# eryxcoop/acvm-backend-plonky2

Hardware: AMD Instinct MI355X
Metric: prove latency (ms) + proofs/sec at 2^20 LDE rows, 1 GPU(s): value = proofs/sec, witness resident in HBM, 4 proof(s) in flight per GPU; latency_ms_single_proof = lone resident proof; *_host_witness = p2gpu_prove from host RAM (PCIe inside the call) (higher is better)
Workload: dtype u64; 1 GPU; synth(d=17,sha): 131072 gates -> 2^20 LDE rows, 234 wires / 80 routed, KeccakGoldilocksConfig, rate 8, cap 2^4, 28 queries, 16 PoW bits (BASELINE configs[2] shape); degree_bits=17, lde_rows=1048576, mix=sha, public_inputs=0, in_flight_per_gpu=4, proof_bytes=170972

## Files before the change

### acvm-backend-plonky2_amd/__init__.py

```python
from .prover import (
    CircuitData,
    WitnessPlan,
    build_blob,
    VerifierCircuitData,
    ProofWithPublicInputs,
    P2GpuError,
    device_info,
    peer_access,
    init,
    host_array,
    host_free,
    ifft_batch,
    lde_batch,
    commit_values,
    hash_rows,
    field_selftest,
    lib_path,
    load_library,
)
from .synth import make_circuit, synth_lib_path
from . import parallel
from . import translate
from . import acir
```

### acvm-backend-plonky2_amd/csrc/circuit.hpp

```cpp
#pragma once
#include "internal.hpp"
#include "poseidon.hpp"
#include "../../include/p2gpu.h"
#include <cstring>
#include <map>
#include <string>
#include <vector>

#include <exception>

struct p2gpu_circuit;
namespace p2 {

void set_err(const char *fmt, ...);
std::string last_error_copy();
void last_error_restore(const std::string &s);

struct HostHasher {
  int kind = 0;
  const gl_t *prc = nullptr;
};
extern thread_local HostHasher g_hh;
inline size_t hh_bytes() { return g_hh.kind ? 32 : 25; }
inline void sponge_permute(gl_t st[12]) {
// ... 16 lines not shown
    } else {
      poseidon_hash_no_pad_host(v, n, d.w, g_hh.prc);
    }
    return d;
  }
  if (n * 8 <= 25) {
    for (size_t i = 0; i < n; i++) d.w[i] = v[i];
    return d;
  }
  uint64_t h[4];
  keccak256_words(v, n, h);
  return dig_from_state(h);
}
inline dig_t node_digest(const dig_t &l, const dig_t &r) {
  if (!g_hh.kind) return keccak_two_to_one(l, r);
  gl_t st[12] = {l.w[0], l.w[1], l.w[2], l.w[3], r.w[0], r.w[1], r.w[2], r.w[3], 0, 0, 0, 0};
  poseidon_permute_host(st, g_hh.prc);
  dig_t d;
  for (int i = 0; i < 4; i++) d.w[i] = st[i];
  return d;
}

struct Challenger {
  gl_t state[12];
  gl_t in[8];
  int n_in = 0;
  gl_t out[8];
  int n_out = 0;
  Challenger() { memset(state, 0, sizeof state); }
  void duplex() {
    for (int i = 0; i < n_in; i++) state[i] = in[i];
    n_in = 0;
    sponge_permute(state);
    for (int i = 0; i < 8; i++) out[i] = state[i];
    n_out = 8;
  }
  void observe(gl_t e) {
    n_out = 0;
    in[n_in++] = e;
    if (n_in == 8) duplex();
  }
  void observe_digest(const dig_t &d) {
    gl_t e[4];
    digest_elems(d, e);
    for (int i = 0; i < 4; i++) observe(e[i]);
  }
  void observe_cap(const std::vector<dig_t> &cap) {
    for (auto &d : cap) observe_digest(d);
  }
  void observe_ext(ext_t e) {
    observe(e.c0);
    observe(e.c1);
  }
  gl_t get() {
    if (n_in != 0 || n_out == 0) duplex();
    return out[--n_out];
  }
  ext_t get_ext() {
    gl_t a = get();
    gl_t b = get();
    return ext_make(a, b);
  }
};

inline dig_t host_hash_no_pad(const std::vector<gl_t> &v) {
  if (g_hh.kind) {
    dig_t d;
    poseidon_hash_no_pad_host(v.data(), v.size(), d.w, g_hh.prc);
    return d;
  }
  uint64_t h[4];
  keccak256_words(v.data(), v.size(), h);
  return dig_from_state(h);
}

template <class T>
struct DBuf {
  T *p = nullptr;
  size_t count = 0;
  hipError_t alloc(size_t n) {
    count = n;
    if (n == 0) return hipSuccess;
    return hipMalloc((void **)&p, n * sizeof(T));
  }
  void release() {
    if (p) (void)hipFree(p);
    p = nullptr;
  }
};

struct PinnedArena {
  uint8_t *base = nullptr;
  size_t cap = 0, used = 0;
  hipError_t alloc(size_t bytes) {
    cap = bytes;
    used = 0;
    return hipHostMalloc((void **)&base, bytes, hipHostMallocDefault);
  }
  void release() {
    if (base) (void)hipHostFree(base);
    base = nullptr;
  }
  void reset() { used = 0; }
  template <class T> T *take(size_t n) {
    const size_t off = (used + 63) & ~(size_t)63, bytes = n * sizeof(T);
    if (!base || off + bytes > cap) return nullptr;
    used = off + bytes;
    return (T *)(base + off);
  }
};

struct Batch {
  uint32_t cols = 0, d = 0;
  uint32_t ncl = 0;
  CosetMap cm;
  DBuf<gl_t> coeffs;
  DBuf<gl_t> lde;
  DBuf<dig_t> dig;
  std::vector<size_t> level_off;
  std::vector<dig_t> cap;
  void release() {
    coeffs.release();
    lde.release();
    dig.release();
  }
};

struct KernelStat {
  double ms = 0, bytes = 0;
  uint64_t launches = 0;
};
struct PendingEv {
  const char *name;
  double bytes;
  hipEvent_t a, b;
};


struct CircuitState {
  uint32_t d, W, R, NC, num_selectors, K, QF, rate_bits, cap_h, pow_bits, num_queries, n_steps, arity[8];
  uint32_t num_gates, num_pi, flags, PP, nchunks;
  uint32_t hasher = 0;
  size_t n, N;
  uint32_t C;
  std::vector<GateDesc> gates;
  std::vector<gl_t> k_is;
  std::vector<uint8_t> blob_prefix;
  uint32_t nterms = 0, max_gate_constraints = 0;
  uint32_t gate_groups = 1;
  uint32_t half_slots = 0;
  uint32_t gate_groups_half = 1;
  uint32_t sums_groups = 1;
  int half_gates = 1;
  bool half_auto = false;
  gl_t half_cross[16];
  DBuf<gl_t> hsum, htmp_a, htmp_b;
  int device = 0;
  hipStream_t stream = nullptr;
  hipStream_t copy_stream = nullptr;
  std::vector<hipEvent_t> copy_events;
  bool wires_ntt_done = false;
  bool wires_hash_done = false;
  DBuf<uint64_t> hash_state;
  DBuf<uint32_t> wire_nz;
  DBuf<gl_t> wire_scalar;
  uint32_t sparse_row = UINT32_MAX;
  SparseRows sparse_rows;
  DBuf<gl_t> sparse_coeffs, sparse_lde;
  DBuf<gl_t> sparse_partial;
  DBuf<uint32_t> wire_nzlist;
  DBuf<uint32_t> wire_clean;
  int zero_columns = 1;
  bool structured_off = false;
  uint32_t last_dense = 0;
  uint32_t gate_wires = 0;
  int virtual_columns = 1;
  DBuf<gl_t> tw_fwd, tw_inv, scale, inv_scale, d_kis, d_sigmas, fri_scale, qconst;
  DBuf<gl_t> l0_lde;
  DBuf<GateDesc> d_gates;
  DBuf<uint8_t> d_row_gate;
  DBuf<gl_t> d_gconsts, d_prc;
  DBuf<gl_t> d_prc_hash;
  NttPlan *plan_inv = nullptr, *plan_fwd = nullptr;
  std::vector<NttPlan *> fri_plans;
  Batch cs, wires, zp, quot;
  dig_t circuit_digest;
  gl_t poseidon_rc[360];
  gl_t poseidon_rc_gate[360];
  DBuf<gl_t> wires_vals, zp_vals, cp, scan_tmp, apow, qvals, qtmp, pw, partial, ext_apow, f01, f01v, fv;
  std::vector<DBuf<gl_t>> fri_coef, fri_vals;
  std::vector<Batch> fri_trees;
  DBuf<unsigned long long> pow_result;
  PinnedArena pin;
  uint64_t *tail_stage = nullptr;
  DBuf<uint64_t> gather_ptrs;
  DBuf<gl_t> gather_out;
  size_t gather_cap = 0;
  std::vector<uint64_t> h_ptrs;
  std::vector<uint8_t> h_out;
  int shard_rank = 0, shard_world = 1;
  p2gpu_allgather_fn shard_fn = nullptr;
  void *shard_ctx = nullptr;
  void *rccl_comm = nullptr;
  int shard_exercise = 0;
  int shard_zs = 0;
  int shard_reduce = 0;
  int shard_intt = 0;
  DBuf<gl_t> xchg_recv;
  std::vector<p2gpu_circuit *> group;
  struct PeerGroup *peer = nullptr;
  uint64_t pow_hint = UINT64_MAX;
  int profile = 0;
  int self_check = 1;
  int blocking_sync = 0;
  hipEvent_t sync_event = nullptr;
  std::map<std::string, KernelStat> kstats;
  std::vector<PendingEv> pending;
  std::vector<hipEvent_t> event_pool;
};

}

#define P2GPU_CATCH                                                   \
  catch (const std::exception &e) {                                   \
    p2::set_err("internal error: %s", e.what());                      \
    return P2GPU_E_DEVICE;                                            \
  }                                                                   \
  catch (...) {                                                       \
    p2::set_err("internal error");                                    \
    return P2GPU_E_DEVICE;                                            \
  }

struct p2gpu_circuit : p2::CircuitState {};

namespace p2 {
extern void (*g_circuit_release)(p2gpu_circuit *);
void use_hasher(const p2gpu_circuit *c);
void shard_assemble_cap(int world, unsigned rate_bits, size_t cap_per, const dig_t *gathered, std::vector<dig_t> &cap);
int circuit_parse(const uint8_t *blob, size_t len, p2gpu_circuit *c, size_t *off, const uint8_t **cap_in);
const char *gate_validate(uint32_t kind, const uint32_t p[4], uint32_t W, uint32_t gate_consts, uint64_t *wires_used,
                          uint32_t *consts_used);
uint32_t gate_num_constraints(uint32_t kind, const uint32_t p[4]);
uint32_t gate_degree(uint32_t kind, const uint32_t p[4]);
struct BuildPlan {
  size_t n = 0, prefix_len = 0;
  uint32_t R = 0, num_selectors = 0, ngc = 0, NC = 0;
  std::vector<uint32_t> gstart, gend, gsel, arity;
};
int build_plan(const p2gpu_build_params *bp, const p2gpu_gate_decl *gates, uint32_t num_gates, bool have_row_constants, BuildPlan &pl);
int build_prefix(const BuildPlan &pl, const p2gpu_build_params *bp, const p2gpu_gate_decl *gates, uint32_t hasher, uint8_t *out);
bool plonk_identity_holds(const p2gpu_circuit *c, const std::vector<ext_t> &op, const gl_t *betas, const gl_t *gammas,
                          const gl_t *alphas, ext_t zeta, const gl_t pih[4]);
}
```

### acvm-backend-plonky2_amd/csrc/gl.hpp

```cpp
#pragma once
#include <cstdint>
#include <cstddef>

#if defined(__HIPCC__)
#include <hip/hip_runtime.h>
#include <type_traits>
#define P2_HD __host__ __device__ __forceinline__
#else
#define P2_HD inline
#endif

namespace p2 {

typedef uint64_t gl_t;
constexpr uint64_t GL_P = 0xFFFFFFFF00000001ULL;
constexpr uint64_t GL_EPS = 0xFFFFFFFFULL;
constexpr uint64_t GL_GEN = 14293326489335486720ULL;
constexpr uint64_t GL_ROOT_2_32 = 7277203076849721926ULL;

#ifndef P2_GL_ASM
#define P2_GL_ASM 1
#endif
#if defined(__HIP_DEVICE_COMPILE__) && P2_GL_ASM
#define P2_GL_DEV_ASM 1
#else
#define P2_GL_DEV_ASM 0
#endif

P2_HD gl_t gl_canon_c(uint64_t x) { return x >= GL_P ? x - GL_P : x; }
P2_HD gl_t gl_add_c(gl_t a, gl_t b) {
  uint64_t s = a + b;
  if (s < a || s >= GL_P) s -= GL_P;
  return s;
}
P2_HD gl_t gl_sub_c(gl_t a, gl_t b) { return a >= b ? a - b : a - b + GL_P; }
P2_HD gl_t gl_reduce128_c(uint64_t lo, uint64_t hi) {
  uint64_t hh = hi >> 32, hl = hi & GL_EPS;
  uint64_t t0 = lo - hh;
  if (lo < hh) t0 -= GL_EPS;
  uint64_t t1 = hl * GL_EPS;
  uint64_t t2 = t0 + t1;
  if (t2 < t1) t2 += GL_EPS;
  return gl_canon_c(t2);
}

#ifndef P2_HZ_A_N
#define P2_HZ_A_N 0
#endif
#ifndef P2_HZ_B_N
#define P2_HZ_B_N 0
#endif
#if P2_HZ_A_N == 0
#define P2_HZ_A ""
#elif P2_HZ_A_N == 1
#define P2_HZ_A "s_nop 0\n\t"
#else
#define P2_HZ_A "s_nop 1\n\t"
#endif
#if P2_HZ_B_N == 0
#define P2_HZ_B ""
#elif P2_HZ_B_N == 1
#define P2_HZ_B "s_nop 0\n\t"
#else
#define P2_HZ_B "s_nop 1\n\t"
#endif
#if P2_GL_DEV_ASM
P2_HD gl_t gl_join(uint32_t lo, uint32_t hi) { return ((uint64_t)hi << 32) | lo; }
P2_HD gl_t gl_canon(uint64_t x) {
  const uint64_t g = __builtin_amdgcn_uicmpl(x, GL_P - 1, 34 );
  uint32_t r0, r1;
  uint64_t junk;
  asm("s_nop 1\n\t"
      "v_subb_co_u32 %0, %2, %3, 0, %5\n\t"
      "v_addc_co_u32 %1, %2, %4, 0, %5"
      : "=&v"(r0), "=&v"(r1), "=&s"(junk)
      : "v"((uint32_t)x), "v"((uint32_t)(x >> 32)), "s"(g));
  return gl_join(r0, r1);
}
P2_HD gl_t gl_sub(gl_t a, gl_t b) {
  uint32_t d0, d1;
  uint64_t k;
  asm("v_sub_co_u32 %0, vcc, %3, %5\n\t"
      "v_subb_co_u32 %1, vcc, %4, %6, vcc\n\t"
      "v_addc_co_u32 %0, %2, %0, 0, vcc\n\t"
      P2_HZ_A "s_andn2_b64 vcc, vcc, %2\n\t" P2_HZ_B
      "v_subb_co_u32 %1, vcc, %1, 0, vcc"
      : "=&v"(d0), "=&v"(d1), "=&s"(k)
      : "v"((uint32_t)a), "v"((uint32_t)(a >> 32)), "v"((uint32_t)b), "v"((uint32_t)(b >> 32))
      : "vcc", "scc");
  return gl_join(d0, d1);
}
P2_HD gl_t gl_add(gl_t a, gl_t b) {
  uint32_t s0, s1;
  uint64_t c;
  asm("v_add_co_u32 %0, vcc, %3, %5\n\t"
      "v_addc_co_u32 %1, %2, %4, %6, vcc"
      : "=&v"(s0), "=&v"(s1), "=&s"(c)
      : "v"((uint32_t)a), "v"((uint32_t)(a >> 32)), "v"((uint32_t)b), "v"((uint32_t)(b >> 32))
      : "vcc");
  const uint64_t m = c | __builtin_amdgcn_uicmpl(gl_join(s0, s1), GL_P - 1, 34);
  uint32_t r0, r1;
  uint64_t k;
  asm("v_subb_co_u32 %0, %2, %3, 0, %5\n\t"
      P2_HZ_A "s_andn2_b64 %2, %5, %2\n\t" P2_HZ_B
      "v_addc_co_u32 %1, %2, %4, 0, %2"
      : "=&v"(r0), "=&v"(r1), "=&s"(k)
      : "v"(s0), "v"(s1), "s"(m)
      : "scc");
  return gl_join(r0, r1);
}
P2_HD uint64_t gl_reduce_words_nc(uint32_t w0, uint32_t w1, uint32_t w2, uint32_t w3) {
  uint32_t r0, r1, y0;
  uint64_t cy, k;
  asm("v_add_co_u32 %1, vcc, %6, %7\n\t"
      "v_addc_co_u32 %2, %3, %7, %8, vcc\n\t"
      "v_addc_co_u32 %1, vcc, %1, 0, vcc\n\t"
      "v_sub_co_u32 %0, vcc, %5, %2\n\t"
      "v_subb_co_u32 %1, vcc, %1, 0, vcc\n\t"
      "v_subb_co_u32 %1, %4, %1, 0, %3\n\t"
      P2_HZ_A "s_or_b64 vcc, vcc, %4\n\t" P2_HZ_B
      "v_addc_co_u32 %0, %4, %0, 0, vcc\n\t"
      P2_HZ_A "s_andn2_b64 vcc, vcc, %4\n\t" P2_HZ_B
      "v_subb_co_u32 %1, vcc, %1, 0, vcc"
      : "=&v"(r0), "=&v"(r1), "=&v"(y0), "=&s"(cy), "=&s"(k)
      : "v"(w0), "v"(w1), "v"(w2), "v"(w3)
      : "vcc", "scc");
  return gl_join(r0, r1);
}
P2_HD gl_t gl_reduce_words(uint32_t w0, uint32_t w1, uint32_t w2, uint32_t w3) { return gl_canon(gl_reduce_words_nc(w0, w1, w2, w3)); }
P2_HD gl_t gl_reduce128(uint64_t lo, uint64_t hi) {
  return gl_reduce_words((uint32_t)lo, (uint32_t)(lo >> 32), (uint32_t)hi, (uint32_t)(hi >> 32));
}
P2_HD gl_t gl_reduce_add_eps(uint32_t w0, uint32_t w1, uint32_t w2) {
  uint32_t r0, r1, t0, t1;
  uint64_t k;
  asm("v_sub_co_u32 %2, vcc, 0, %7\n\t"
      "v_subbrev_co_u32 %3, vcc, 0, %7, vcc\n\t"
      "v_add_co_u32 %0, vcc, %5, %2\n\t"
      "v_addc_co_u32 %1, vcc, %6, %3, vcc\n\t"
      "v_subb_co_u32 %0, %4, %0, 0, vcc\n\t"
      P2_HZ_A "s_andn2_b64 vcc, vcc, %4\n\t" P2_HZ_B
      "v_addc_co_u32 %1, vcc, %1, 0, vcc"
      : "=&v"(r0), "=&v"(r1), "=&v"(t0), "=&v"(t1), "=&s"(k)
      : "v"(w0), "v"(w1), "v"(w2)
      : "vcc", "scc");
  return gl_canon(gl_join(r0, r1));
}
P2_HD gl_t gl_reduce_eps_sub(uint32_t z, uint32_t h0, uint32_t h1) {
  uint32_t r0, r1, t0, t1;
  uint64_t k;
  asm("v_sub_co_u32 %2, vcc, 0, %7\n\t"
      "v_subbrev_co_u32 %3, vcc, 0, %7, vcc\n\t"
      "v_sub_co_u32 %0, vcc, %2, %5\n\t"
      "v_subb_co_u32 %1, vcc, %3, %6, vcc\n\t"
      "v_addc_co_u32 %0, %4, %0, 0, vcc\n\t"
      P2_HZ_A "s_andn2_b64 vcc, vcc, %4\n\t" P2_HZ_B
      "v_subb_co_u32 %1, vcc, %1, 0, vcc"
      : "=&v"(r0), "=&v"(r1), "=&v"(t0), "=&v"(t1), "=&s"(k)
      : "v"(h0), "v"(h1), "v"(z)
      : "vcc", "scc");
  return gl_canon(gl_join(r0, r1));
}
#else
P2_HD gl_t gl_canon(uint64_t x) { return gl_canon_c(x); }
P2_HD gl_t gl_add(gl_t a, gl_t b) { return gl_add_c(a, b); }
P2_HD gl_t gl_sub(gl_t a, gl_t b) { return gl_sub_c(a, b); }
P2_HD gl_t gl_reduce128(uint64_t lo, uint64_t hi) { return gl_reduce128_c(lo, hi); }
#endif
#if defined(__HIPCC__)
template <class T>
__device__ __forceinline__ T ld_uniform(const T *p) {
#if defined(__HIP_DEVICE_COMPILE__)
  typedef const T __attribute__((address_space(4))) *cptr;
  return *(cptr)(uintptr_t)p;
#else
  return *p;
#endif
}
#endif
P2_HD gl_t gl_neg(gl_t a) { return a ? GL_P - a : 0; }
P2_HD gl_t gl_dbl(gl_t a) { return gl_add(a, a); }

#if defined(__HIP_DEVICE_COMPILE__)
__device__ __forceinline__ void gl_mul128(uint64_t a, uint64_t b, uint64_t &lo, uint64_t &hi) {
  const uint32_t a0 = (uint32_t)a, a1 = (uint32_t)(a >> 32), b0 = (uint32_t)b, b1 = (uint32_t)(b >> 32);
  uint64_t p0, m, p3, cdummy, carry;
  uint32_t r1, r2, r3;
  asm("v_mad_u64_u32 %0, %3, %5, %6, 0\n\t"
      "v_mad_u64_u32 %1, %3, %5, %8, 0\n\t"
      "v_mad_u64_u32 %2, %3, %7, %8, 0\n\t"
      "v_mad_u64_u32 %1, %4, %7, %6, %1"
      : "=&v"(p0), "=&v"(m), "=&v"(p3), "=&s"(cdummy), "=&s"(carry)
      : "v"(a0), "v"(b0), "v"(a1), "v"(b1));
  asm("v_add_co_u32 %0, vcc, %3, %4\n\t"
      "v_addc_co_u32 %1, vcc, %5, %6, vcc\n\t"
      "v_addc_co_u32 %2, vcc, %7, 0, vcc\n\t"
      "v_addc_co_u32 %2, vcc, %2, 0, %8"
      : "=&v"(r1), "=&v"(r2), "=&v"(r3)
      : "v"((uint32_t)(p0 >> 32)), "v"((uint32_t)m), "v"((uint32_t)p3), "v"((uint32_t)(m >> 32)),
        "v"((uint32_t)(p3 >> 32)), "s"(carry)
      : "vcc");
  lo = ((uint64_t)r1 << 32) | (uint32_t)p0;
  hi = ((uint64_t)r3 << 32) | r2;
}
#endif
P2_HD gl_t gl_mul(gl_t a, gl_t b) {
#if defined(__HIP_DEVICE_COMPILE__)
  uint64_t lo, hi;
  gl_mul128(a, b, lo, hi);
#else
  unsigned __int128 x = (unsigned __int128)a * b;
  uint64_t lo = (uint64_t)x, hi = (uint64_t)(x >> 64);
#endif
  return gl_reduce128(lo, hi);
}
P2_HD gl_t gl_sqr(gl_t a) { return gl_mul(a, a); }
#if defined(__HIP_DEVICE_COMPILE__) && P2_GL_DEV_ASM
__device__ __forceinline__ uint64_t gl_mul_nc(uint64_t a, uint64_t b) {
  uint64_t lo, hi;
  gl_mul128(a, b, lo, hi);
  return gl_reduce_words_nc((uint32_t)lo, (uint32_t)(lo >> 32), (uint32_t)hi, (uint32_t)(hi >> 32));
}
__device__ __forceinline__ uint64_t gl_reduce128_nc(uint64_t lo, uint64_t hi) {
  return gl_reduce_words_nc((uint32_t)lo, (uint32_t)(lo >> 32), (uint32_t)hi, (uint32_t)(hi >> 32));
}
#else
P2_HD uint64_t gl_mul_nc(uint64_t a, uint64_t b) { return gl_mul(gl_canon(a), gl_canon(b)); }
P2_HD uint64_t gl_reduce128_nc(uint64_t lo, uint64_t hi) { return gl_reduce128(lo, hi); }
#endif
P2_HD gl_t gl_mul_add(gl_t a, gl_t b, gl_t c) {
#if defined(__HIP_DEVICE_COMPILE__)
  uint64_t lo, hi;
  gl_mul128(a, b, lo, hi);
  lo += c;
  hi += lo < c;
#else
  unsigned __int128 x = (unsigned __int128)a * b + c;
  uint64_t lo = (uint64_t)x, hi = (uint64_t)(x >> 64);
#endif
  return gl_reduce128(lo, hi);
}
P2_HD uint64_t gl_mul_add_nc(uint64_t a, uint64_t b, gl_t c) {
#if defined(__HIP_DEVICE_COMPILE__)
  uint64_t lo, hi;
  gl_mul128(a, b, lo, hi);
  lo += c;
  hi += lo < c;
  return gl_reduce128_nc(lo, hi);
#else
  return gl_mul_add(gl_canon(a), gl_canon(b), c);
#endif
}
P2_HD gl_t gl_mul_small(gl_t a, uint32_t k) {
#if defined(__HIP_DEVICE_COMPILE__)
  uint64_t lo = a * (uint64_t)k;
  uint64_t hi = __umul64hi(a, (uint64_t)k);
#else
  unsigned __int128 x = (unsigned __int128)a * k;
  uint64_t lo = (uint64_t)x, hi = (uint64_t)(x >> 64);
#endif
  uint64_t t1 = hi * GL_EPS;
  uint64_t t2 = lo + t1;
  if (t2 < t1) t2 += GL_EPS;
  return gl_canon(t2);
}
#if defined(__HIPCC__)
struct Acc160 {
  uint32_t w[5];
  __device__ __forceinline__ void clear() { w[0] = w[1] = w[2] = w[3] = w[4] = 0; }
  __device__ __forceinline__ void mac(gl_t a, gl_t c) {
#if defined(__HIP_DEVICE_COMPILE__)
    uint64_t lo, hi;
    gl_mul128(a, c, lo, hi);
    asm("v_add_co_u32 %0, vcc, %0, %5\n\t"
        "v_addc_co_u32 %1, vcc, %1, %6, vcc\n\t"
        "v_addc_co_u32 %2, vcc, %2, %7, vcc\n\t"
        "v_addc_co_u32 %3, vcc, %3, %8, vcc\n\t"
        "v_addc_co_u32 %4, vcc, 0, %4, vcc"
        : "+v"(w[0]), "+v"(w[1]), "+v"(w[2]), "+v"(w[3]), "+v"(w[4])
        : "v"((uint32_t)lo), "v"((uint32_t)(lo >> 32)), "v"((uint32_t)hi), "v"((uint32_t)(hi >> 32))
        : "vcc");
#else
    (void)a; (void)c;
#endif
  }
  __device__ __forceinline__ gl_t value() const {
    const gl_t r = gl_reduce128(((uint64_t)w[1] << 32) | w[0], ((uint64_t)w[3] << 32) | w[2]);
    return gl_sub(r, (uint64_t)w[4] << 32);
  }
};
#endif
P2_HD gl_t gl_pow(gl_t b, uint64_t e) {
  gl_t r = 1;
  while (e) {
    if (e & 1) r = gl_mul(r, b);
    b = gl_sqr(b);
    e >>= 1;
  }
  return r;
}
P2_HD gl_t gl_sqr_n(gl_t a, int k) {
  for (int i = 0; i < k; i++) a = gl_mul(a, a);
  return a;
}
P2_HD gl_t gl_inv(gl_t a) {
  const gl_t e2 = gl_mul(gl_mul(a, a), a);
  const gl_t e4 = gl_mul(gl_sqr_n(e2, 2), e2);
  const gl_t e8 = gl_mul(gl_sqr_n(e4, 4), e4);
  const gl_t e16 = gl_mul(gl_sqr_n(e8, 8), e8);
  const gl_t e24 = gl_mul(gl_sqr_n(e16, 8), e8);
  const gl_t e28 = gl_mul(gl_sqr_n(e24, 4), e4);
  const gl_t e30 = gl_mul(gl_sqr_n(e28, 2), e2);
  const gl_t e31 = gl_mul(gl_mul(e30, e30), a);
  const gl_t e32 = gl_mul(gl_mul(e31, e31), a);
  return gl_mul(gl_sqr_n(e31, 33), e32);
}
P2_HD gl_t gl_root(unsigned k) {
  gl_t g = GL_ROOT_2_32;
  for (unsigned i = k; i < 32; i++) g = gl_sqr(g);
  return g;
}
// ... 107 lines not shown
```

### acvm-backend-plonky2_amd/csrc/handle.hip

```cpp
#include "prover_internal.hpp"
#include <functional>

using namespace p2;

namespace {

void release_for_destroy(p2gpu_circuit *c) {
  for (p2gpu_circuit *m : c->group) {
    m->peer = nullptr;
    release_for_destroy(m);
    delete m;
  }
  c->group.clear();
  if (c->peer && c->shard_rank == 0) {
    for (auto e : c->peer->recv_free) if (e) (void)hipEventDestroy(e);
    for (auto e : c->peer->sent) if (e) (void)hipEventDestroy(e);
    delete c->peer;
  }
  c->peer = nullptr;
  (void)hipSetDevice(c->device);
  if (c->stream) (void)hipStreamSynchronize(c->stream);
  if (c->rccl_comm) (void)rccl().CommDestroy((ncclComm_t)c->rccl_comm);
  c->rccl_comm = nullptr;
  circuit_release(c);
}
struct ReleaseHook {
  ReleaseHook() { p2::g_circuit_release = release_for_destroy; }
} g_release_hook;

struct Scratch {
  std::vector<void *> ptrs;
  hipStream_t st = nullptr;
  ~Scratch() {
    for (void *p : ptrs) (void)hipFree(p);
    if (st) (void)hipStreamDestroy(st);
  }
  template <class T> T *alloc(size_t n) {
    void *p = nullptr;
    if (hipMalloc(&p, (n ? n : 1) * sizeof(T)) != hipSuccess) return nullptr;
    ptrs.push_back(p);
    return (T *)p;
  }
};

}

namespace p2 {

int g_device = -1;
std::vector<int> g_peer_access;
std::vector<int> g_devices;

void circuit_release(p2gpu_circuit *c) {
  c->tw_fwd.release(); c->tw_inv.release(); c->scale.release(); c->inv_scale.release(); c->d_kis.release();
  c->d_sigmas.release(); c->fri_scale.release(); c->d_gates.release(); c->qconst.release(); c->l0_lde.release();
  c->d_row_gate.release(); c->d_gconsts.release(); c->d_prc.release(); c->d_prc_hash.release();
  c->hsum.release(); c->htmp_a.release(); c->htmp_b.release();
  c->cs.release(); c->wires.release(); c->zp.release(); c->quot.release();
  c->wires_vals.release(); c->zp_vals.release(); c->cp.release(); c->scan_tmp.release();
  c->apow.release(); c->qvals.release(); c->qtmp.release(); c->pw.release(); c->partial.release();
  c->ext_apow.release(); c->f01.release(); c->f01v.release(); c->fv.release();
  for (auto &b : c->fri_coef) b.release();
  for (auto &b : c->fri_vals) b.release();
  for (auto &b : c->fri_trees) b.release();
  c->hash_state.release();
  c->wire_nz.release();
  c->wire_nzlist.release();
  c->wire_clean.release();
  c->wire_scalar.release(); c->sparse_coeffs.release(); c->sparse_lde.release(); c->sparse_partial.release();
  c->pin.release();
  if (c->sync_event) (void)hipEventDestroy(c->sync_event);
  c->sync_event = nullptr;
  if (c->tail_stage) (void)hipHostFree(c->tail_stage);
  c->tail_stage = nullptr;
  c->pow_result.release(); c->gather_ptrs.release(); c->gather_out.release(); c->xchg_recv.release();
  ntt_plan_destroy(c->plan_inv);
  ntt_plan_destroy(c->plan_fwd);
  for (auto *p : c->fri_plans)
    if (p != c->plan_fwd) ntt_plan_destroy(p);
  c->plan_inv = c->plan_fwd = nullptr;
  c->fri_plans.clear();
  for (auto e : c->event_pool) (void)hipEventDestroy(e);
  for (auto e : c->copy_events) (void)hipEventDestroy(e);
  if (c->copy_stream) (void)hipStreamDestroy(c->copy_stream);
  if (c->stream) (void)hipStreamDestroy(c->stream);
}

int ensure_device() {
  if (g_device >= 0) return 0;
  int cnt = 0;
  hipError_t e = hipGetDeviceCount(&cnt);
  if (e != hipSuccess || cnt == 0) {
    set_err("no HIP device available (%s); libp2gpu has no CPU fallback", e == hipSuccess ? "count=0" : hipGetErrorString(e));
    return P2GPU_E_DEVICE;
  }
  int dev = 0;
  (void)hipGetDevice(&dev);
  g_device = dev;
  g_devices.assign(1, dev);
  g_peer_access.assign(1, -1);
  return 0;
}

}


namespace {

#define CK(e, what)                                       \
  do {                                                    \
    const hipError_t e_ = (e);                            \
    if (e_ != hipSuccess) {                               \
      set_err("%s: %s", what, hipGetErrorString(e_));     \
      return P2GPU_E_DEVICE;                              \
    }                                                     \
  } while (0)

void schedule_gates(p2gpu_circuit *c) {
  c->nterms = c->K + c->K * c->nchunks + c->max_gate_constraints;
  auto cost = [](const GateDesc &g) { return g.kind == G_POSEIDON ? 0u : 4u * g.num_constraints + 8u; };
  const uint32_t perm_cost = (uint32_t)env_uint("P2GPU_PERM_COST", 8u * c->R + 100u);
  uint32_t total = 0;
  for (auto &g : c->gates) total += cost(g);
  c->gate_groups = env_uint("P2GPU_GATE_GROUPS", total > 2 * perm_cost ? 4u : 1u) == 4 ? 4u : 1u;
  uint32_t load[4] = {perm_cost, 0, 0, 0};
  std::vector<uint32_t> order(c->gates.size());
  for (size_t i = 0; i < order.size(); i++) order[i] = (uint32_t)i;
  std::sort(order.begin(), order.end(), [&](uint32_t x, uint32_t y) { return cost(c->gates[x]) > cost(c->gates[y]); });
  for (uint32_t gi : order) {
    uint32_t best = 0;
    for (uint32_t q = 1; q < 4; q++)
      if (load[q] < load[best]) best = q;
    c->gates[gi].pad = c->gate_groups == 4 ? best : 0;
    load[best] += cost(c->gates[gi]);
  }
  uint64_t half_constraints = 0;
  if (env_flag("P2GPU_HALF_GATES", true) && c->d >= 6 && c->rate_bits == 3)
    for (auto &g : c->gates)
      if (g.kind != G_POSEIDON && g.num_constraints >= 48 && gate_degree(g.kind, g.p) <= 4 && c->half_slots < 64) {
        g.pad |= (++c->half_slots) << 16;
        half_constraints += g.num_constraints;
      }
  c->half_auto = (half_constraints << c->d) >= ((uint64_t)12 << 20);
  if (c->half_slots) {
    auto cost_main = [&](const GateDesc &g) { return gate_half_slot(g) ? 8u : cost(g); };
    uint32_t rest = 0;
    for (auto &g : c->gates) rest += cost_main(g);
    c->gate_groups_half = env_uint("P2GPU_GATE_GROUPS_HALF", rest > 2 * perm_cost ? 4u : 1u) == 4 ? 4u : 1u;
    uint32_t lm[4] = {perm_cost, 0, 0, 0}, ls[4] = {0, 0, 0, 0};
    c->sums_groups = env_uint("P2GPU_SUMS_GROUPS", c->half_slots >= 2 ? 4u : 1u) == 4 ? 4u : 1u;
    for (uint32_t gi : order) {
      GateDesc &g = c->gates[gi];
      uint32_t bm = 0, bs = 0;
      for (uint32_t q = 1; q < 4; q++) {
        if (lm[q] < lm[bm]) bm = q;
        if (ls[q] < ls[bs]) bs = q;
      }
      if (c->gate_groups_half == 4) g.pad |= bm << 4;
      lm[bm] += cost_main(g);
      if (gate_half_slot(g)) {
        if (c->sums_groups == 4) g.pad |= bs << 8;
        ls[bs] += cost(g);
      }
    }
  }
}

int make_streams(p2gpu_circuit *c) {
  if (poseidon_upload_constants()) { set_err("uploading Poseidon constants failed"); return P2GPU_E_DEVICE; }
  CK(hipStreamCreateWithFlags(&c->stream, hipStreamNonBlocking), "hipStreamCreate");
  CK(hipStreamCreateWithFlags(&c->copy_stream, hipStreamNonBlocking), "hipStreamCreate");
  return P2GPU_OK;
}

int make_root_tables(p2gpu_circuit *c) {
  hipStream_t st = c->stream;
  const size_t n = c->n;
  const uint32_t d = c->d, K = c->K, C = c->C;
  const size_t half = n >= 2 ? n / 2 : 1;
  CK(c->tw_fwd.alloc(half), "alloc tw");
  CK(c->tw_inv.alloc(half), "alloc tw");
  CK(c->scale.alloc((size_t)C * n), "alloc scale");
  CK(c->inv_scale.alloc((size_t)C * n), "alloc scale");
  CK(c->fri_scale.alloc((size_t)C * n), "alloc scale");
  CK(c->d_kis.alloc(c->R), "alloc kis");
  CK(c->d_sigmas.alloc((size_t)c->R * n), "alloc sigmas");
  CK(c->d_gates.alloc(c->num_gates ? c->num_gates : 1), "alloc gates");
  gl_t wn = gl_root(d), wN = gl_root(d + c->rate_bits);
  c->plan_inv = ntt_plan_create(st, d, NttDir::ToCoeffs);
  c->plan_fwd = ntt_plan_create(st, d, NttDir::ToValues);
  if (!c->plan_inv || !c->plan_fwd) { set_err("ntt plan allocation failed"); return P2GPU_E_DEVICE; }
  fill_powers(st, c->tw_fwd.p, wn, (uint32_t)half);
  fill_powers(st, c->tw_inv.p, gl_inv(wn), (uint32_t)half);
  fill_coset_scale(st, c->scale.p, GL_GEN, wN, d, C, 1);
  fill_coset_scale(st, c->inv_scale.p, gl_inv(GL_GEN), gl_inv(wN), d, C, 1);
  if (c->half_slots) {
    const size_t per = (size_t)4 * c->half_slots * K * n;
    CK(c->hsum.alloc(2 * per), "alloc gate sums");
    CK(c->htmp_a.alloc(per), "alloc gate sums");
    CK(c->htmp_b.alloc(per), "alloc gate sums");
    const gl_t w8 = gl_root(3), quarter = gl_inv(4);
    for (int mo = 0; mo < 4; mo++)
      for (int m = 0; m < 4; m++) {
        const gl_t base = gl_pow(w8, (uint64_t)((2 * mo + 1 - 2 * m + 16) % 8));
        gl_t acc = 0, pw = 1;
        for (int j = 0; j < 4; j++) {
          acc = gl_add(acc, pw);
          pw = gl_mul(pw, base);
        }
        c->half_cross[4 * mo + m] = gl_mul(acc, quarter);
      }
  }
  CK(c->qconst.alloc(24), "alloc qconst");
  {
    gl_t qc[24];
    memset(qc, 0, sizeof qc);
    gl_t wC = gl_root(c->rate_bits), gn = gl_pow(GL_GEN, n);
    for (uint32_t r = 0; r < C; r++) {
      qc[r] = gl_mul(GL_GEN, gl_pow(wN, r));
      qc[8 + r] = gl_sub(gl_mul(gn, gl_pow(wC, r)), 1);
      qc[16 + r] = gl_inv(qc[8 + r]);
    }
    CK(hipMemcpy(c->qconst.p, qc, sizeof qc, hipMemcpyHostToDevice), "copy qconst");
    CK(c->l0_lde.alloc((size_t)C * n), "alloc L0 table");
    fill_l0_table(st, c->qconst.p, c->tw_fwd.p, 0, d, C, gl_inv((gl_t)n), c->l0_lde.p);
  }
  return P2GPU_OK;
}

int tables_from_blob(p2gpu_circuit *c, const gl_t *constants, const gl_t *sigmas) {
  const size_t n = c->n;
  const uint32_t ngc = c->NC - c->num_selectors;
  CK(hipMemcpyAsync(c->d_sigmas.p, sigmas, 8 * (size_t)c->R * n, hipMemcpyHostToDevice, c->stream), "copy sigmas");
  std::vector<uint8_t> rg(n, 0);
  for (size_t row = 0; row < n; row++) {
    uint32_t gi = 0;
    for (uint32_t s = 0; s < c->num_selectors; s++) {
      gl_t v = constants[(size_t)s * n + row];
      if (c->num_selectors == 1 || v != 0xFFFFFFFFULL) gi = (uint32_t)v;
    }
    if (gi >= c->num_gates) { set_err("selector column holds an unknown gate index"); return P2GPU_E_BLOB; }
    rg[row] = (uint8_t)gi;
    if (c->sparse_row == UINT32_MAX && c->gates[gi].kind == G_PUBLIC_INPUT) c->sparse_row = (uint32_t)row;
  }
  c->sparse_rows = SparseRows();
  if (c->sparse_row != UINT32_MAX) {
    c->sparse_rows.row[c->sparse_rows.count++] = c->sparse_row;
    for (size_t row = 0; row < n && c->sparse_rows.count < MAX_SPARSE_ROWS; row++)
      if (c->gates[rg[row]].kind == G_POSEIDON) c->sparse_rows.row[c->sparse_rows.count++] = (uint32_t)row;
  }
  CK(hipMemcpy(c->d_row_gate.p, rg.data(), n, hipMemcpyHostToDevice), "copy row_gate");
  if (ngc)
    CK(hipMemcpy(c->d_gconsts.p, constants + (size_t)c->num_selectors * n, 8 * (size_t)ngc * n, hipMemcpyHostToDevice), "copy gconsts");
  return P2GPU_OK;
}

int alloc_proof_buffers(p2gpu_circuit *c) {
  hipStream_t st = c->stream;
  const size_t n = c->n;
  const uint32_t d = c->d, K = c->K, C = c->C;
  const uint32_t ncs = c->NC + c->R, nzp = K * (1 + c->PP), nq = K * c->QF;
  const uint32_t nall = ncs + c->W + nzp + nq;
  if (batch_alloc(c, c->cs, ncs) || batch_alloc(c, c->wires, c->W) || batch_alloc(c, c->zp, nzp) || batch_alloc(c, c->quot, nq)) return P2GPU_E_DEVICE;
  CK(c->wires_vals.alloc((size_t)c->W * n), "alloc wires");
  CK(c->wire_nz.alloc(c->W), "alloc wire flags");
  CK(c->wire_nzlist.alloc(c->W + 1), "alloc wire flags");
  CK(c->wire_clean.alloc(c->W), "alloc wire flags");
  CK(hipMemsetAsync(c->wire_clean.p, 0, sizeof(uint32_t) * c->W, c->stream), "clear wire flags");
  CK(c->wire_scalar.alloc((size_t)MAX_SPARSE_ROWS * c->W), "alloc wire flags");
  if (c->sparse_row != UINT32_MAX) {
    const uint32_t nr = c->sparse_rows.count;
    CK(c->sparse_coeffs.alloc((size_t)nr * n), "alloc sparse basis");
// ... 267 lines not shown


int p2gpu_circuit_create_on(const uint8_t *blob, size_t len, int device_id, p2gpu_circuit **out_c) try {
  if (!blob || !out_c) return P2GPU_E_ARG;
  if (int rc = ensure_device()) return rc;
  if (std::find(g_devices.begin(), g_devices.end(), device_id) == g_devices.end()) {
    set_err("p2gpu_circuit_create_on: device %d is not in the list given to p2gpu_init", device_id);
    return P2GPU_E_ARG;
  }
  const int rc = circuit_create_one(blob, len, device_id, out_c);
  (void)hipSetDevice(g_device);
  return rc;
} P2GPU_CATCH

static int circuit_make(const std::function<int(int, p2gpu_circuit **)> &one, p2gpu_circuit **out_c) {
  if (g_devices.size() <= 1) return one(g_device, out_c);
  const int n = (int)g_devices.size();
  std::vector<p2gpu_circuit *> hs(n, nullptr);
  std::vector<int> rcs(n, 0);
  std::vector<std::string> errs(n);
  {
    std::vector<std::thread> th;
    for (int q = 0; q < n; q++)
      th.emplace_back([&, q] {
        rcs[q] = one(g_devices[q], &hs[q]);
        if (rcs[q]) errs[q] = p2gpu_last_error();
      });
    for (auto &t : th) t.join();
  }
  (void)hipSetDevice(g_device);
  auto drop = [&](int rc, const std::string &msg) {
    for (auto *h : hs)
      if (h) {
        h->peer = nullptr;
        p2gpu_circuit_destroy(h);
      }
    set_err("%s", msg.c_str());
    return rc;
  };
  for (int q = 0; q < n; q++)
    if (rcs[q]) return drop(rcs[q], errs[q]);
  for (int q = 0; q < n; q++) {
    if (int rc = shard_args_ok(hs[q], q, n)) return drop(rc, p2gpu_last_error());
    if (int rc = shard_layout(hs[q], q, n)) return drop(rc, p2gpu_last_error());
  }
  PeerGroup *pg = new PeerGroup();
  pg->n = n;
  pg->cs = hs;
  pg->recv_free.assign(n, nullptr);
  pg->sent.assign(n, nullptr);
  pg->proof_scratch.resize(n);
  pg->send_ptr.resize(n);
  pg->recv_ptr.resize(n);
  for (int q = 0; q < n; q++) {
    (void)hipSetDevice(hs[q]->device);
    if (hipEventCreateWithFlags(&pg->recv_free[q], hipEventDisableTiming) != hipSuccess ||
        hipEventCreateWithFlags(&pg->sent[q], hipEventDisableTiming) != hipSuccess) {
      for (int k = 0; k <= q; k++) {
        (void)hipSetDevice(hs[k]->device);
        if (pg->recv_free[k]) (void)hipEventDestroy(pg->recv_free[k]);
        if (pg->sent[k]) (void)hipEventDestroy(pg->sent[k]);
        hs[k]->peer = nullptr;
      }
      (void)hipSetDevice(g_device);
      delete pg;
      return drop(P2GPU_E_DEVICE, "hipEventCreate failed");
    }
    hs[q]->peer = pg;
  }
  (void)hipSetDevice(g_device);
  for (int q = 1; q < n; q++) hs[0]->group.push_back(hs[q]);
  *out_c = hs[0];
  return P2GPU_OK;
}

int p2gpu_circuit_create(const uint8_t *blob, size_t len, p2gpu_circuit **out_c) try {
  if (!blob || !out_c) return P2GPU_E_ARG;
  if (int rc = ensure_device()) return rc;
  return circuit_make([&](int device, p2gpu_circuit **h) { return circuit_create_one(blob, len, device, h); }, out_c);
} P2GPU_CATCH


int p2gpu_circuit_build_on(const p2gpu_build_params *bp, const p2gpu_gate_decl *gates, uint32_t num_gates, const uint32_t *row_gate,
                           const uint64_t *row_constants, const uint32_t *copies, size_t num_copies, uint32_t hasher, int device_id,
                           p2gpu_circuit **out_c) try {
  BuildCall b;
  if (int rc = build_call_prepare(b, bp, gates, num_gates, row_gate, row_constants, copies, num_copies, hasher, out_c)) return rc;
  if (int rc = ensure_device()) return rc;
  if (std::find(g_devices.begin(), g_devices.end(), device_id) == g_devices.end()) {
    set_err("p2gpu_circuit_build_on: device %d is not in the list given to p2gpu_init", device_id);
    return P2GPU_E_ARG;
  }
  const int rc = circuit_build_one(b, device_id, out_c);
  (void)hipSetDevice(g_device);
  return rc;
} P2GPU_CATCH

int p2gpu_circuit_build(const p2gpu_build_params *bp, const p2gpu_gate_decl *gates, uint32_t num_gates, const uint32_t *row_gate,
                        const uint64_t *row_constants, const uint32_t *copies, size_t num_copies, uint32_t hasher, p2gpu_circuit **out_c) try {
  BuildCall b;
  if (int rc = build_call_prepare(b, bp, gates, num_gates, row_gate, row_constants, copies, num_copies, hasher, out_c)) return rc;
  if (int rc = ensure_device()) return rc;
  return circuit_make([&](int device, p2gpu_circuit **h) { return circuit_build_one(b, device, h); }, out_c);
} P2GPU_CATCH

int p2gpu_circuit_export_blob(const p2gpu_circuit *cc, uint8_t *out, size_t *len) try {
  if (!cc || !len) return P2GPU_E_ARG;
  if (int rc = prover_handle(cc)) return rc;
  p2gpu_circuit *c = const_cast<p2gpu_circuit *>(cc);
  const size_t n = c->n, nsel = c->num_selectors, ngc = c->NC - c->num_selectors;
  const size_t need = c->blob_prefix.size() + 8 * ((size_t)c->NC + c->R) * n;
  if (!out || *len < need) {
    const bool probe = out == nullptr;
    *len = need;
    if (probe) return P2GPU_OK;
    set_err("blob buffer too small: need %zu bytes", need);
    return P2GPU_E_BUFFER;
  }
  HIP_TRY(hipSetDevice(c->device));
  Scratch S;
  gl_t *sel = S.alloc<gl_t>(nsel * n);
  if (!sel) { set_err("hipMalloc failed"); (void)hipSetDevice(g_device); return P2GPU_E_DEVICE; }
  build_selector_columns(c->stream, c, sel);
  memcpy(out, c->blob_prefix.data(), c->blob_prefix.size());
  uint8_t *q = out + c->blob_prefix.size();
  hipError_t e = hipMemcpyAsync(q, sel, 8 * nsel * n, hipMemcpyDeviceToHost, c->stream);
  if (e == hipSuccess && ngc) e = hipMemcpyAsync(q + 8 * nsel * n, c->d_gconsts.p, 8 * ngc * n, hipMemcpyDeviceToHost, c->stream);
  if (e == hipSuccess) e = hipMemcpyAsync(q + 8 * (size_t)c->NC * n, c->d_sigmas.p, 8 * (size_t)c->R * n, hipMemcpyDeviceToHost, c->stream);
  const hipError_t e2 = hipStreamSynchronize(c->stream);
  (void)hipSetDevice(g_device);
  HIP_TRY(e);
  HIP_TRY(e2);
  *len = need;
  return P2GPU_OK;
} P2GPU_CATCH




int p2gpu_circuit_set(p2gpu_circuit *c, const char *key, uint64_t value) try {
  if (!c || !key) return P2GPU_E_ARG;
  if (int rc = prover_handle(c)) return rc;
  for (p2gpu_circuit *m : c->group)
    if (int rc = p2gpu_circuit_set(m, key, value)) return rc;
  HIP_TRY(hipSetDevice(c->device));
  std::string k(key);
  if (k == "pow_hint") c->pow_hint = value;
  else if (k == "self_check") c->self_check = (int)value;
  else if (k == "shard_exercise") c->shard_exercise = (int)value;
  else if (k == "shard_intt") c->shard_intt = (int)value;
  else if (k == "shard_reduce") c->shard_reduce = (int)value;
  else if (k == "shard_zs") c->shard_zs = (int)value;
  else if (k == "half_gates") c->half_gates = (int)value;
  else if (k == "blocking_sync") c->blocking_sync = (int)value;
  else if (k == "virtual_columns") {
    c->virtual_columns = (int)value;
    if (c->wire_clean.p) HIP_TRY(hipMemsetAsync(c->wire_clean.p, 0, sizeof(uint32_t) * c->W, c->stream));
  }
  else if (k == "zero_columns") {
    c->zero_columns = (int)value;
    c->structured_off = false;
    if (c->wire_clean.p) HIP_TRY(hipMemsetAsync(c->wire_clean.p, 0, sizeof(uint32_t) * c->W, c->stream));
  }
  else if (k == "profile") {
    flush_kstats(c);
    c->profile = (int)value;
    c->kstats.clear();
  } else {
    set_err("unknown knob %s", key);
    return P2GPU_E_ARG;
  }
  return P2GPU_OK;
} P2GPU_CATCH

static int shard_layout(p2gpu_circuit *c, int rank, int world) {
  HIP_TRY(hipSetDevice(c->device));
  if (c->stream) HIP_TRY(hipStreamSynchronize(c->stream));
  if (c->rccl_comm) {
    (void)rccl().CommDestroy((ncclComm_t)c->rccl_comm);
    c->rccl_comm = nullptr;
  }
  c->shard_rank = rank;
  c->shard_world = world;
  c->shard_fn = nullptr;
  c->shard_ctx = nullptr;
  const uint32_t ncl = c->C / (uint32_t)world;
  const size_t cap_per = ((size_t)1 << c->cap_h) >> c->rate_bits;
  CosetMap cm;
  cm.first = (uint32_t)rank;
  cm.stride = (uint32_t)world;
  Batch *bs[3] = {&c->wires, &c->zp, &c->quot};
  for (Batch *b : bs) {
    b->ncl = ncl;
    b->cm = cm;
    tree_layout(*b, ncl, c->n, cap_per);
  }
  if (c->n_steps > 0) {
    Batch &t0 = c->fri_trees[0];
    t0.ncl = ncl;
    t0.cm = cm;
    tree_layout(t0, ncl, c->n >> c->arity[0], cap_per);
  }
  if (c->wire_clean.p) HIP_TRY(hipMemsetAsync(c->wire_clean.p, 0, sizeof(uint32_t) * c->W, c->stream));
  c->xchg_recv.release();
  HIP_TRY(c->xchg_recv.alloc(std::max({(size_t)world * c->gather_cap, (size_t)c->K * c->C * c->n, (size_t)2 * world * c->n}) + 64));
  return P2GPU_OK;
}
static int shard_args_ok(p2gpu_circuit *c, int rank, int world) {
  if (!c || world < 1 || rank < 0 || rank >= world || (c->C % (uint32_t)world) != 0) {
    set_err("bad shard configuration: rank %d of %d (cosets %u)", rank, world, c ? c->C : 0u);
    return P2GPU_E_ARG;
  }
  if (int rc = prover_handle(c)) return rc;
  return P2GPU_OK;
}

static int not_a_group(const p2gpu_circuit *c) {
  if (c && c->peer) { set_err("this handle is a device group of one process (p2gpu_init with several ids): its sharding is fixed"); return P2GPU_E_ARG; }
  return P2GPU_OK;
}
int p2gpu_circuit_set_shard(p2gpu_circuit *c, int rank, int world, p2gpu_allgather_fn fn, void *ctx) try {
  if (int rc = not_a_group(c)) return rc;
  if (int rc = shard_args_ok(c, rank, world)) return rc;
  if (world > 1 && !fn) { set_err("a host all-gather callback is needed for world > 1 (or use p2gpu_circuit_set_shard_rccl)"); return P2GPU_E_ARG; }
  if (int rc = shard_layout(c, rank, world)) return rc;
  c->shard_fn = fn;
  c->shard_ctx = ctx;
  return P2GPU_OK;
} P2GPU_CATCH

int p2gpu_shard_unique_id(uint8_t id_out[128]) try {
  if (!id_out) return P2GPU_E_ARG;
  if (int rc = ensure_device()) return rc;
  if (!rccl().ok) { set_err("librccl.so.1 could not be loaded"); return P2GPU_E_DEVICE; }
  ncclUniqueId id;
  static_assert(sizeof id == 128, "ncclUniqueId is 128 bytes");
  RCCL_TRY(rccl().GetUniqueId(&id));
  memcpy(id_out, &id, sizeof id);
  return P2GPU_OK;
} P2GPU_CATCH

int p2gpu_circuit_set_shard_rccl(p2gpu_circuit *c, int rank, int world, const uint8_t id_in[128]) try {
  if (int rc = not_a_group(c)) return rc;
  if (int rc = shard_args_ok(c, rank, world)) return rc;
  if (!id_in) return P2GPU_E_ARG;
  if (!rccl().ok) { set_err("librccl.so.1 could not be loaded"); return P2GPU_E_DEVICE; }
  if (int rc = shard_layout(c, rank, world)) return rc;
  ncclUniqueId id;
  memcpy(&id, id_in, sizeof id);
  ncclComm_t comm = nullptr;
  RCCL_TRY(rccl().CommInitRank(&comm, world, id, rank));
  c->rccl_comm = (void *)comm;
  return P2GPU_OK;
} P2GPU_CATCH

int p2gpu_kernel_stats(p2gpu_circuit *c, char *names, double *ms, double *bytes, uint64_t *launches, int cap) try {
  if (!c) return P2GPU_E_ARG;
  if (int rc = prover_handle(c)) return rc;
  (void)hipSetDevice(c->device);
  (void)hipStreamSynchronize(c->stream);
  flush_kstats(c);
  int i = 0;
  for (auto &kv : c->kstats) {
    if (i >= cap) break;
    snprintf(names + 64 * i, 64, "%s", kv.first.c_str());
    ms[i] = kv.second.ms;
    bytes[i] = kv.second.bytes;
    launches[i] = kv.second.launches;
    i++;
  }
  return i;
} P2GPU_CATCH

int p2gpu_ifft_batch(const uint64_t *vals, size_t ncols, unsigned d, uint64_t *coeffs_out) try {
  if (int rc = ensure_device()) return rc;
  if (!vals || !coeffs_out || d > 24) return P2GPU_E_ARG;
  Scratch S;
  HIP_TRY(hipStreamCreate(&S.st));
  size_t n = (size_t)1 << d, half = n >= 2 ? n / 2 : 1;
  gl_t *a = S.alloc<gl_t>(ncols * n), *b = S.alloc<gl_t>(ncols * n), *tw = S.alloc<gl_t>(half);
  if (!a || !b || !tw) { set_err("hipMalloc failed"); return P2GPU_E_DEVICE; }
  HIP_TRY(hipMemcpyAsync(a, vals, 8 * ncols * n, hipMemcpyHostToDevice, S.st));
  NttPlan *plan = ntt_plan_create(S.st, d, NttDir::ToCoeffs);
  if (!plan) { set_err("hipMalloc failed"); return P2GPU_E_DEVICE; }
  ntt_batch(S.st, plan, a, b, (uint32_t)ncols, 1, nullptr, gl_inv((gl_t)n), false);
  bitrev_cols(S.st, b, a, d, (uint32_t)ncols);
  hipError_t e1 = hipMemcpyAsync(coeffs_out, a, 8 * ncols * n, hipMemcpyDeviceToHost, S.st);
  hipError_t e2 = hipStreamSynchronize(S.st);
  ntt_plan_destroy(plan);
  HIP_TRY(e1);
  HIP_TRY(e2);
  return P2GPU_OK;
} P2GPU_CATCH

int p2gpu_lde_batch(const uint64_t *coeffs, size_t ncols, unsigned d, unsigned rate_bits, uint64_t *lde_out) try {
  if (int rc = ensure_device()) return rc;
  if (!coeffs || !lde_out || d > 24 || rate_bits > 3) return P2GPU_E_ARG;
  Scratch S;
  HIP_TRY(hipStreamCreate(&S.st));
  size_t n = (size_t)1 << d, half = n >= 2 ? n / 2 : 1;
  uint32_t C = 1u << rate_bits;
  gl_t *a = S.alloc<gl_t>(ncols * n), *b = S.alloc<gl_t>(ncols * n), *tw = S.alloc<gl_t>(half);
  gl_t *scale = S.alloc<gl_t>(C * n), *lde = S.alloc<gl_t>(C * ncols * n);
  if (!a || !b || !tw || !scale || !lde) { set_err("hipMalloc failed"); return P2GPU_E_DEVICE; }
  HIP_TRY(hipMemcpyAsync(a, coeffs, 8 * ncols * n, hipMemcpyHostToDevice, S.st));
  bitrev_cols(S.st, a, b, d, (uint32_t)ncols);
  NttPlan *plan = ntt_plan_create(S.st, d, NttDir::ToValues);
  if (!plan) { set_err("hipMalloc failed"); return P2GPU_E_DEVICE; }
  fill_coset_scale(S.st, scale, GL_GEN, gl_root(d + rate_bits), d, C, 1);
  ntt_batch(S.st, plan, b, lde, (uint32_t)ncols, C, scale, 1, false);
  std::vector<gl_t> tmp(C * ncols * n);
  hipError_t e1 = hipMemcpyAsync(tmp.data(), lde, 8 * tmp.size(), hipMemcpyDeviceToHost, S.st);
  hipError_t e2 = hipStreamSynchronize(S.st);
  ntt_plan_destroy(plan);
  HIP_TRY(e1);
  HIP_TRY(e2);
  for (uint32_t r = 0; r < C; r++)
    for (size_t col = 0; col < ncols; col++)
      for (size_t k = 0; k < n; k++) lde_out[col * C * n + C * k + r] = tmp[((size_t)r * ncols + col) * n + k];
  return P2GPU_OK;
} P2GPU_CATCH

static int field_selftest_words(const uint64_t *a, const uint64_t *b, size_t n, uint64_t *bad_out, size_t words);
int p2gpu_field_selftest(const uint64_t *a, const uint64_t *b, size_t n, uint64_t bad_out[8]) { return field_selftest_words(a, b, n, bad_out, 8); }
int p2gpu_field_selftest16(const uint64_t *a, const uint64_t *b, size_t n, uint64_t bad_out[16]) { return field_selftest_words(a, b, n, bad_out, 16); }
static int field_selftest_words(const uint64_t *a, const uint64_t *b, size_t n, uint64_t *bad_out, size_t words) try {
  if (int rc = ensure_device()) return rc;
  if (!a || !b || !bad_out || n == 0 || n > ((size_t)1 << 28)) return P2GPU_E_ARG;
  Scratch S;
  HIP_TRY(hipStreamCreate(&S.st));
  uint64_t *da = S.alloc<uint64_t>(n), *db = S.alloc<uint64_t>(n);
  unsigned long long *bad = S.alloc<unsigned long long>(16);
  if (!da || !db || !bad) { set_err("hipMalloc failed"); return P2GPU_E_DEVICE; }
  HIP_TRY(hipMemcpyAsync(da, a, 8 * n, hipMemcpyHostToDevice, S.st));
  HIP_TRY(hipMemcpyAsync(db, b, 8 * n, hipMemcpyHostToDevice, S.st));
  HIP_TRY(hipMemsetAsync(bad, 0, 128, S.st));
  field_selftest(S.st, da, db, (uint32_t)n, bad);
  HIP_TRY(hipMemcpyAsync(bad_out, bad, 8 * words, hipMemcpyDeviceToHost, S.st));
  HIP_TRY(hipStreamSynchronize(S.st));
  return P2GPU_OK;
} P2GPU_CATCH

int p2gpu_hash_rows(const uint64_t *rows, size_t n_rows, size_t row_len, uint8_t *digests_out) try {
  if (int rc = ensure_device()) return rc;
  if (!rows || !digests_out) return P2GPU_E_ARG;
  Scratch S;
  HIP_TRY(hipStreamCreate(&S.st));
  gl_t *a = S.alloc<gl_t>(n_rows * row_len);
  dig_t *dg = S.alloc<dig_t>(n_rows);
  if (!a || !dg) { set_err("hipMalloc failed"); return P2GPU_E_DEVICE; }
  HIP_TRY(hipMemcpyAsync(a, rows, 8 * n_rows * row_len, hipMemcpyHostToDevice, S.st));
  hash_rows(S.st, a, n_rows, (uint32_t)row_len, dg);
  std::vector<dig_t> h(n_rows);
  HIP_TRY(hipMemcpyAsync(h.data(), dg, sizeof(dig_t) * n_rows, hipMemcpyDeviceToHost, S.st));
  HIP_TRY(hipStreamSynchronize(S.st));
  for (size_t i = 0; i < n_rows; i++) memcpy(digests_out + 25 * i, h[i].w, 25);
  return P2GPU_OK;
} P2GPU_CATCH

int p2gpu_commit_values(const uint64_t *vals, size_t ncols, unsigned d, unsigned rate_bits, unsigned cap_h,
                        uint8_t *cap_out) try {
  if (int rc = ensure_device()) return rc;
  if (!vals || !cap_out || d > 24 || rate_bits > 3 || cap_h < rate_bits || cap_h > rate_bits + d) return P2GPU_E_ARG;
  HalfBuilt own(new p2gpu_circuit());
  p2gpu_circuit *c = own.get();
  c->d = d; c->rate_bits = rate_bits; c->cap_h = cap_h; c->n = (size_t)1 << d; c->N = c->n << rate_bits;
  c->C = 1u << rate_bits; c->device = g_device; c->n_steps = 0;
  int rc = P2GPU_OK;
  size_t n = c->n, half = n >= 2 ? n / 2 : 1;
  do {
    if (hipStreamCreate(&c->stream) != hipSuccess || c->tw_fwd.alloc(half) != hipSuccess ||
        c->tw_inv.alloc(half) != hipSuccess || c->scale.alloc((size_t)c->C * n) != hipSuccess ||
        c->wires_vals.alloc(ncols * n) != hipSuccess || c->pin.alloc(((size_t)1 << 16) + 2 * (sizeof(dig_t) << cap_h)) != hipSuccess) {
      set_err("hipMalloc failed");
      rc = P2GPU_E_DEVICE;
      break;
    }
    if ((rc = batch_alloc(c, c->wires, (uint32_t)ncols))) break;
    c->plan_inv = ntt_plan_create(c->stream, d, NttDir::ToCoeffs);
    c->plan_fwd = ntt_plan_create(c->stream, d, NttDir::ToValues);
    if (!c->plan_inv || !c->plan_fwd) {
      set_err("hipMalloc failed");
      rc = P2GPU_E_DEVICE;
      break;
    }
    fill_coset_scale(c->stream, c->scale.p, GL_GEN, gl_root(d + rate_bits), d, c->C, 1);
    if (hipMemcpyAsync(c->wires_vals.p, vals, 8 * ncols * n, hipMemcpyHostToDevice, c->stream) != hipSuccess) {
      set_err("copy failed");
      rc = P2GPU_E_DEVICE;
      break;
    }
    if ((rc = batch_commit_from_values(c, c->wires, c->wires_vals.p))) break;
    for (size_t i = 0; i < c->wires.cap.size(); i++) memcpy(cap_out + 25 * i, c->wires.cap[i].w, 25);
  } while (0);
  return rc;
} P2GPU_CATCH

}
```

### acvm-backend-plonky2_amd/csrc/internal.hpp

```cpp
#pragma once
#include <hip/hip_runtime.h>
#include <cstdlib>
#include <vector>
#include "gl.hpp"
#include "keccak.hpp"
#include "gates.hpp"

namespace p2 {

constexpr int MAX_GATES = 64;
constexpr uint32_t MAX_GATE_CONSTRAINTS = 4096;
constexpr uint32_t MAX_ARITY_BITS = 4;
constexpr int MAX_CHALLENGES = 2;
constexpr int MAX_ROUTED = 128;

inline bool env_flag(const char *name, bool dflt) {
  const char *e = getenv(name);
  return e && *e ? *e != '0' : dflt;
}
inline uint64_t env_uint(const char *name, uint64_t dflt) {
  const char *e = getenv(name);
  return e ? strtoull(e, nullptr, 10) : dflt;
}

struct Prof {
  virtual void begin(const char *kernel, double algorithmic_bytes) = 0;
  virtual void end() = 0;
  virtual ~Prof() {}
};
extern thread_local Prof *g_prof;
struct ProfScope {
  ProfScope(const char *k, double bytes) { if (g_prof) g_prof->begin(k, bytes); }
  ~ProfScope() { if (g_prof) g_prof->end(); }
};

constexpr uint32_t MAX_SPARSE_ROWS = 4;
struct SparseRows {
  uint32_t row[MAX_SPARSE_ROWS] = {UINT32_MAX, UINT32_MAX, UINT32_MAX, UINT32_MAX};
  uint32_t count = 0;
};
struct ColHints {
  const uint32_t *cls = nullptr;
  const uint32_t *clean = nullptr;
  const gl_t *val = nullptr;
  const gl_t *basis = nullptr;
  bool basis_per_coset = false;
  uint32_t nrows = 1, val_stride = 0;
  size_t basis_stride = 0;
  uint32_t virt_first = UINT32_MAX;
  uint32_t dense_hint = 0;
  bool fill_only = false;
};
void column_clean_update(hipStream_t st, const uint32_t *cls, uint32_t cols, uint32_t *clean, bool after);
void column_flags(hipStream_t st, const gl_t *vals, uint32_t cols, uint32_t d, const SparseRows &rows, uint32_t *flags,
                  gl_t *scalar, uint32_t sstride);

constexpr int NTT_MAX_ROUNDS = 6;
enum class NttDir { ToCoeffs, ToValues };
struct NttPass {
  uint32_t s, a, tb, nrounds;
  uint32_t r[NTT_MAX_ROUNDS], tw_off[NTT_MAX_ROUNDS];
  bool direct = false;
  uint32_t rm = 0, rl = 0, fold_r = 0, fold_s0 = 0;
  uint32_t ftw_off = 0;
};
struct NttPlan {
  uint32_t d = 0;
  NttDir dir = NttDir::ToCoeffs;
  std::vector<NttPass> passes;
  gl_t *ptw = nullptr;
  size_t table_len = 0;
};
struct CosetMap {
  uint32_t first = 0, stride = 1;
};
NttPlan *ntt_plan_create(hipStream_t st, uint32_t d, NttDir dir);
void ntt_plan_destroy(NttPlan *p);
void ntt_batch(hipStream_t st, const NttPlan *plan, const gl_t *src, gl_t *dst, uint32_t cols, uint32_t cosets,
               const gl_t *scale, gl_t post, bool src_per_coset, CosetMap cm = CosetMap(), uint32_t stride_cols = 0,
               const ColHints *hints = nullptr);

void fill_powers(hipStream_t st, gl_t *out, gl_t root, uint32_t count);
void fill_coset_scale(hipStream_t st, gl_t *out, gl_t shift, gl_t wN, uint32_t d, uint32_t cosets, gl_t mult);

void bitrev_cols(hipStream_t st, const gl_t *in, gl_t *out, uint32_t d, uint32_t cols);
void field_selftest(hipStream_t st, const uint64_t *a, const uint64_t *b, uint32_t n, unsigned long long *bad);

struct VirtCols {
  const uint32_t *cls = nullptr;
  const gl_t *val = nullptr;
  const gl_t *basis = nullptr;
  uint32_t first = UINT32_MAX;
  uint32_t coset_first = 0, coset_stride = 1;
};
uint32_t hash_lde_leaves(hipStream_t st, const gl_t *lde, uint32_t cols, uint32_t d, uint32_t cosets, dig_t *dig, const gl_t *prc = nullptr,
                         const VirtCols *virt = nullptr, dig_t *lvl1 = nullptr, dig_t *lvl2 = nullptr);
void hash_lde_absorb(hipStream_t st, const gl_t *lde, uint32_t cols, uint32_t d, uint32_t cosets, uint32_t blk0,
                     uint32_t nblk, bool first, bool last, uint64_t *state, dig_t *dig, const VirtCols *virt = nullptr);
void hash_rows(hipStream_t st, const gl_t *rows, size_t n_rows, uint32_t row_len, dig_t *dig);
void hash_fri_leaves(hipStream_t st, const gl_t *vals, uint32_t lg_npc, uint32_t cosets, uint32_t arity_bits,
                     dig_t *dig, const gl_t *prc = nullptr);
bool tree_levels(hipStream_t st, dig_t *lvl, uint32_t cosets, uint32_t m, uint32_t cap_per, const gl_t *prc = nullptr,
                 dig_t *host_mirror = nullptr);

struct ZsArgs {
  const gl_t *wires;
  const gl_t *sigmas;
  const gl_t *k_is;
  const gl_t *sub_tw;
  uint32_t tw_shift;
  uint32_t d, R, QF, nchunks, K;
  gl_t betas[MAX_CHALLENGES], gammas[MAX_CHALLENGES];
  gl_t *cp;
  uint32_t sb;
  uint32_t row0, rows;
  gl_t *zp;
};
void zs_partial_products(hipStream_t st, const ZsArgs &a, gl_t *scan_tmp);
void zs_chunks(hipStream_t st, const ZsArgs &a);
void zs_scan_finish(hipStream_t st, const ZsArgs &a, gl_t *scan_tmp);

struct QuotArgs {
  const gl_t *cs_lde;
  const gl_t *wires_lde;
  const gl_t *zp_lde;
  const gl_t *k_is;
  const gl_t *tw;
  const gl_t *apow;
  const GateDesc *gates;
  const GateDesc *host_gates;
  gl_t *out;
  uint32_t tw_shift, d, rate_bits, W, R, NC, num_selectors, K, QF, nchunks, PP, num_gates, nterms, has_poseidon;
  uint32_t gate_groups;
  uint32_t gate_groups_half;
  uint32_t use_half;
  uint32_t nsk;
  gl_t *hsum;
  uint32_t coset_first, coset_stride, ncosets;
  gl_t betas[MAX_CHALLENGES], gammas[MAX_CHALLENGES];
  gl_t pi_hash[4];
  const gl_t *qconst;
  gl_t n_inv;
  const gl_t *l0;
};
void quotient_eval(hipStream_t st, const QuotArgs &a);
void gate_sums_eval(hipStream_t st, const QuotArgs &a, uint32_t groups);
void gate_sums_cross(hipStream_t st, const gl_t *in, const gl_t *inv_scale, gl_t *out, uint32_t d, uint32_t cols, const gl_t F[16]);
void fill_l0_table(hipStream_t st, const gl_t *qconst, const gl_t *tw, uint32_t tw_shift, uint32_t d, uint32_t cosets, gl_t n_inv, gl_t *out);
int poseidon_upload_constants();
void quotient_chunks(hipStream_t st, const gl_t *in, const gl_t *inv_scale, gl_t *out, uint32_t d, uint32_t K,
                     uint32_t rate_bits, gl_t w_inv, gl_t gn_inv, gl_t rate_inv, uint32_t world = 1);

void fill_witness(hipStream_t st, gl_t *wires, const uint8_t *row_gate, const GateDesc *gates, const gl_t *gconsts,
                  const gl_t *prc, uint32_t d, uint32_t ngc, uint32_t num_wires);

void ext_powers_bitrev2(hipStream_t st, ext_t base0, ext_t base1, uint32_t d, gl_t *out0, gl_t *out1);
void eval_columns(hipStream_t st, const gl_t *coeffs, uint32_t cols, uint32_t d, const gl_t *pw, uint32_t parts,
                  gl_t *partial , const ColHints *hints = nullptr, const gl_t *basis_partial = nullptr);
struct EvalSegs {
  struct Seg {
    const gl_t *coeffs;
    const gl_t *pw;
    gl_t *partial;
    uint32_t cols;
  } seg[6];
  uint32_t count = 0, hinted = UINT32_MAX;
  const uint32_t *cls = nullptr;
  const gl_t *val = nullptr, *basis_partial = nullptr;
};
void eval_columns_multi(hipStream_t st, const EvalSegs &S, uint32_t d, uint32_t parts, uint32_t col0 = 0, uint32_t ncols = UINT32_MAX);
void reduce_columns(hipStream_t st, const gl_t *coeffs, uint32_t cols, uint32_t d, const gl_t *apow ,
                    uint32_t j0, gl_t *acc, bool accumulate, const uint32_t *nzlist = nullptr, const gl_t *basis = nullptr,
                    const gl_t *fold = nullptr);
void compact_nonzero(hipStream_t st, const uint32_t *flags, uint32_t cols, uint32_t *list);
void sum_parts(hipStream_t st, const gl_t *parts, uint32_t nparts, size_t len, gl_t *out);
void class1_fold(hipStream_t st, const ColHints &h, uint32_t cols, const gl_t *apow, uint32_t j0, gl_t *fold);
void fri_quotient_values(hipStream_t st, const gl_t *F0, const gl_t *F1, uint32_t d, const gl_t *tw, uint32_t tw_shift,
                         ext_t zeta, ext_t gzeta, ext_t f0z, ext_t f1z, ext_t aK, gl_t *out );
void fri_fold(hipStream_t st, const gl_t *in , uint32_t d, uint32_t arity_bits, ext_t beta, gl_t *out);
void pow_search(hipStream_t st, const gl_t state[12], uint32_t pos, uint32_t pow_bits, uint64_t base, uint64_t count,
                unsigned long long *result, const gl_t *prc = nullptr);
void gather_u64(hipStream_t st, const uint64_t *addr, uint32_t count, gl_t *out);

}
```

### acvm-backend-plonky2_amd/csrc/plonk.hip

```cpp
#include "internal.hpp"
#include "gates.hpp"

namespace p2 {

__constant__ gl_t c_poseidon_rc[360];
int poseidon_upload_constants() {
  gl_t rc[360];
  poseidon_round_constants_host(rc);
  gl_t dev[360];
  poseidon_device_constants(rc, dev);
  return hipMemcpyToSymbol(HIP_SYMBOL(c_poseidon_rc), dev, sizeof dev) == hipSuccess ? 0 : -1;
}

__device__ __forceinline__ gl_t root_pow(const gl_t *tw, uint32_t shift, uint32_t d, uint32_t i) {
  uint32_t half = 1u << (d - 1);
  if (d == 0) return 1;
  return i < half ? tw[(size_t)i << shift] : gl_neg(tw[(size_t)(i - half) << shift]);
}

__device__ __forceinline__ size_t zs_idx(const ZsArgs &a, uint32_t col, uint32_t i) {
  const uint32_t cols = a.K * (a.nchunks + 1);
  return ((((size_t)(i >> a.sb) * cols + col) << a.sb) | (i & ((1u << a.sb) - 1u)));
}
__global__ __launch_bounds__(256) void zs_chunk_kernel(ZsArgs a) {
  const uint32_t n = 1u << a.d;
  const uint32_t i = a.row0 + blockIdx.x * blockDim.x + threadIdx.x;
  const uint32_t c = blockIdx.y;
  if (i >= a.row0 + a.rows) return;
  const gl_t x = root_pow(a.sub_tw, a.tw_shift, a.d, i);
  const gl_t beta = a.betas[c], gamma = a.gammas[c];
  const gl_t bx = gl_mul(beta, x);
  gl_t np[16], dp[16];
  for (uint32_t m = 0; m < a.nchunks; m++) {
    uint64_t pn = 1, pd = 1;
    for (uint32_t j = m * a.QF; j < (m + 1) * a.QF && j < a.R; j++) {
      gl_t wv = a.wires[(size_t)j * n + i];
      const gl_t wg = gl_add(wv, gamma);
      const uint64_t num = gl_mul_add_nc(bx, a.k_is[j], wg);
      const uint64_t den = gl_mul_add_nc(beta, a.sigmas[(size_t)j * n + i], wg);
      pn = gl_mul_nc(pn, num);
      pd = gl_mul_nc(pd, den);
    }
    np[m] = gl_canon(pn);
    dp[m] = gl_canon(pd);
  }
  gl_t pre[16];
  gl_t acc = 1;
  for (uint32_t m = 0; m < a.nchunks; m++) {
    pre[m] = acc;
    acc = gl_mul(acc, dp[m]);
  }
  gl_t inv = gl_inv(acc);
  gl_t rowp = 1;
  for (uint32_t m = a.nchunks; m-- > 0;) {
    gl_t di = gl_mul(inv, pre[m]);
    inv = gl_mul(inv, dp[m]);
    gl_t q = gl_mul(np[m], di);
    a.cp[zs_idx(a, c * a.nchunks + m, i)] = q;
    rowp = gl_mul(rowp, q);
  }
  a.cp[zs_idx(a, a.K * a.nchunks + c, i)] = rowp;
}

__device__ __forceinline__ gl_t block_scan_mul(gl_t v, gl_t *lds, gl_t *total) {
  const uint32_t t = threadIdx.x, nt = blockDim.x;
  lds[t] = v;
  __syncthreads();
  for (uint32_t off = 1; off < nt; off <<= 1) {
    gl_t x = lds[t];
    gl_t y = t >= off ? lds[t - off] : 1;
    __syncthreads();
    lds[t] = gl_mul(x, y);
    __syncthreads();
  }
  gl_t incl = lds[t];
  gl_t excl = t ? lds[t - 1] : 1;
  *total = lds[nt - 1];
  (void)incl;
  return excl;
}

__global__ __launch_bounds__(256) void scan_local_kernel(const ZsArgs a, uint32_t n, gl_t *local, gl_t *bsum, uint32_t nblocks) {
  __shared__ gl_t lds[256];
  const uint32_t i = blockIdx.x * blockDim.x + threadIdx.x;
  const uint32_t c = blockIdx.y;
  gl_t v = i < n ? a.cp[zs_idx(a, a.K * a.nchunks + c, i)] : 1;
  gl_t total;
  gl_t excl = block_scan_mul(v, lds, &total);
  if (i < n) local[(size_t)c * n + i] = excl;
  if (threadIdx.x == 0) bsum[(size_t)c * nblocks + blockIdx.x] = total;
}
__global__ __launch_bounds__(1024) void scan_blocks_kernel(gl_t *bsum, uint32_t nblocks) {
  __shared__ gl_t lds[1024];
  const uint32_t c = blockIdx.x;
  gl_t *b = bsum + (size_t)c * nblocks;
  const uint32_t per = (nblocks + blockDim.x - 1) / blockDim.x;
  const uint32_t lo = threadIdx.x * per;
  gl_t prod = 1;
  for (uint32_t j = lo; j < lo + per && j < nblocks; j++) prod = gl_mul(prod, b[j]);
  gl_t total;
  gl_t excl = block_scan_mul(prod, lds, &total);
  gl_t acc = excl;
  for (uint32_t j = lo; j < lo + per && j < nblocks; j++) {
    gl_t v = b[j];
    b[j] = acc;
    acc = gl_mul(acc, v);
  }
}
__global__ __launch_bounds__(256) void zs_finish_kernel(ZsArgs a, const gl_t *local, const gl_t *bpre,
                                                        uint32_t nblocks) {
  const uint32_t n = 1u << a.d;
  const uint32_t i = blockIdx.x * blockDim.x + threadIdx.x;
  const uint32_t c = blockIdx.y;
  if (i >= n) return;
  const uint32_t PP = a.nchunks - 1;
  gl_t z = gl_mul(bpre[(size_t)c * nblocks + blockIdx.x], local[(size_t)c * n + i]);
  a.zp[(size_t)c * n + i] = z;
  gl_t acc = z;
  for (uint32_t m = 0; m < PP; m++) {
    acc = gl_mul(acc, a.cp[zs_idx(a, c * a.nchunks + m, i)]);
    a.zp[((size_t)a.K + (size_t)c * PP + m) * n + i] = acc;
  }
}

void zs_chunks(hipStream_t st, const ZsArgs &a) {
  if (!a.rows) return;
  ProfScope ps("zs_chunk_kernel", 8.0 * a.K * (double)a.rows * (2.0 * a.R + a.nchunks + 1));
  hipLaunchKernelGGL(zs_chunk_kernel, dim3((a.rows + 255) / 256, a.K), dim3(256), 0, st, a);
}
void zs_scan_finish(hipStream_t st, const ZsArgs &a, gl_t *scan_tmp) {
  const uint32_t n = 1u << a.d;
  const uint32_t threads = 256;
  const uint32_t nblocks = (n + threads - 1) / threads;
  gl_t *local = scan_tmp;
  gl_t *bsum = scan_tmp + (size_t)a.K * n;
  ProfScope ps2("zs_scan_finish", 8.0 * a.K * (double)n * (2.0 * a.nchunks + 4));
  hipLaunchKernelGGL(scan_local_kernel, dim3(nblocks, a.K), dim3(threads), 0, st, a, n, local, bsum, nblocks);
  hipLaunchKernelGGL(scan_blocks_kernel, dim3(a.K), dim3(1024), 0, st, bsum, nblocks);
  hipLaunchKernelGGL(zs_finish_kernel, dim3(nblocks, a.K), dim3(threads), 0, st, a, local, bsum, nblocks);
}
void zs_partial_products(hipStream_t st, const ZsArgs &a, gl_t *scan_tmp) {
  zs_chunks(st, a);
  zs_scan_finish(st, a, scan_tmp);
}

struct Consumer {
  Acc160 acc0, acc1;
  const gl_t *ap0, *ap1;
  uint32_t t;
  __device__ __forceinline__ void emit(gl_t c) {
    acc0.mac(ap0[t], c);
    acc1.mac(ap1[t], c);
    t++;
  }
};

#ifndef P2_QUOT_WAVES
#define P2_QUOT_WAVES 6
#endif
template <bool POSEIDON, int G>
__global__ __launch_bounds__(256, P2_QUOT_WAVES) void quotient_kernel(const QuotArgs a) {
  __shared__ gl_t red[2][G > 1 ? G : 1][G > 1 ? 64 : 1];
  const uint32_t grp = G > 1 ? threadIdx.y : 0;
  const uint32_t n = 1u << a.d;
  const uint32_t k = blockIdx.x * blockDim.x + threadIdx.x;
  const uint32_t z = blockIdx.y;
  const uint32_t r = a.coset_first + z * a.coset_stride;
  if (k >= n) return;
  const uint32_t ncs = a.NC + a.R, nzp = a.K * (1 + a.PP);
  const gl_t *cs = a.cs_lde + (size_t)r * ncs * n + k;
  const gl_t *wl = a.wires_lde + (size_t)z * a.W * n + k;
  const gl_t *zl = a.zp_lde + (size_t)z * nzp * n;
  const uint32_t kn = (k + 1) & (n - 1);
  const gl_t x = gl_mul(a.qconst[r], root_pow(a.tw, a.tw_shift, a.d, k));
  Consumer out;
  out.acc0.clear();
  out.acc1.clear();
  out.ap0 = a.apow;
  out.ap1 = a.apow + a.nterms;
  out.t = 0;
  if (grp == 0) {
  const gl_t l0 = a.l0[(size_t)r * n + k];
  for (uint32_t c = 0; c < a.K; c++) out.emit(gl_mul(l0, gl_sub(zl[(size_t)c * n + k], 1)));
  {
    const gl_t bx0 = gl_mul(a.betas[0], x), bx1 = gl_mul(a.betas[1], x);
    const uint32_t t_base = out.t;
    for (uint32_t m = 0; m < a.nchunks; m++) {
      uint64_t n0, d0, n1 = 1, d1 = 1;
      {
        const uint32_t j = m * a.QF;
        const gl_t wv = wl[(size_t)j * n];
        const gl_t sg = cs[(size_t)(a.NC + j) * n];
        const gl_t kj = a.k_is[j];
        const gl_t wg0 = gl_add(wv, a.gammas[0]);
        n0 = gl_mul_add_nc(bx0, kj, wg0);
        d0 = gl_mul_add_nc(a.betas[0], sg, wg0);
        if (a.K > 1) {
          const gl_t wg1 = gl_add(wv, a.gammas[1]);
          n1 = gl_mul_add_nc(bx1, kj, wg1);
          d1 = gl_mul_add_nc(a.betas[1], sg, wg1);
        }
      }
#pragma unroll 7
      for (uint32_t j = m * a.QF + 1; j < (m + 1) * a.QF && j < a.R; j++) {
        const gl_t wv = wl[(size_t)j * n];
        const gl_t sg = cs[(size_t)(a.NC + j) * n];
        const gl_t kj = a.k_is[j];
        const gl_t wg0 = gl_add(wv, a.gammas[0]);
        n0 = gl_mul_nc(n0, gl_mul_add_nc(bx0, kj, wg0));
        d0 = gl_mul_nc(d0, gl_mul_add_nc(a.betas[0], sg, wg0));
        if (a.K > 1) {
          const gl_t wg1 = gl_add(wv, a.gammas[1]);
          n1 = gl_mul_nc(n1, gl_mul_add_nc(bx1, kj, wg1));
          d1 = gl_mul_nc(d1, gl_mul_add_nc(a.betas[1], sg, wg1));
        }
      }
      for (uint32_t c = 0; c < a.K; c++) {
        const gl_t prev = m == 0 ? zl[(size_t)c * n + k] : zl[((size_t)a.K + c * a.PP + m - 1) * n + k];
        const gl_t next = m == a.nchunks - 1 ? zl[(size_t)c * n + kn] : zl[((size_t)a.K + c * a.PP + m) * n + k];
        const gl_t term = c == 0 ? gl_sub(gl_mul(prev, n0), gl_mul(next, d0)) : gl_sub(gl_mul(prev, n1), gl_mul(next, d1));
        out.t = t_base + c * a.nchunks + m;
        out.emit(term);
      }
    }
    out.t = t_base + a.K * a.nchunks;
  }
  }
  const uint32_t t_gates = a.K + a.K * a.nchunks;
  gl_t tot0 = out.acc0.value(), tot1 = out.acc1.value();
  auto W = [&](uint32_t c) { return wl[(size_t)c * n]; };
  auto LC = [&](uint32_t i) { return cs[(size_t)(a.num_selectors + i) * n]; };
  for (uint32_t gi = 0; gi < a.num_gates; gi++) {
    const GateDesc g = a.gates[gi];
    if (g.num_constraints == 0) continue;
    if (!POSEIDON && g.kind == G_POSEIDON) continue;
    if (G > 1 && gate_group(g, a.use_half) != grp) continue;
    const gl_t s = cs[(size_t)g.sel_index * n];
    const gl_t f = gate_filter<BaseOps>(g, gi, a.num_selectors, s);
    if (const uint32_t slot1 = a.use_half ? gate_half_slot(g) : 0u) {
      const gl_t *h = a.hsum + ((size_t)((r & 1u) * 4u + (r >> 1)) * a.nsk + (size_t)(slot1 - 1) * a.K) * n + k;
      tot0 = gl_mul_add(f, h[0], tot0);
      if (a.K > 1) tot1 = gl_mul_add(f, h[n], tot1);
      continue;
    }
    out.acc0.clear();
    out.acc1.clear();
    out.t = t_gates;
    eval_gate<BaseOps, POSEIDON>(g, W, LC, a.pi_hash, c_poseidon_rc, out);
    tot0 = gl_add(tot0, gl_mul(f, out.acc0.value()));
    tot1 = gl_add(tot1, gl_mul(f, out.acc1.value()));
  }
  if constexpr (G > 1) {
    red[0][grp][threadIdx.x] = tot0;
    red[1][grp][threadIdx.x] = tot1;
    __syncthreads();
    if (grp != 0) return;
    for (int q = 1; q < G; q++) {
      tot0 = gl_add(tot0, red[0][q][threadIdx.x]);
      tot1 = gl_add(tot1, red[1][q][threadIdx.x]);
    }
  }
  const gl_t zi = a.qconst[16 + r];
  a.out[((size_t)0 * a.ncosets + z) * n + k] = gl_mul(tot0, zi);
  if (a.K > 1) a.out[((size_t)1 * a.ncosets + z) * n + k] = gl_mul(tot1, zi);
}

#ifndef P2_SUMS_WAVES
#define P2_SUMS_WAVES 8
#endif
template <int G, bool STAGE>
__global__ __launch_bounds__(256, P2_SUMS_WAVES) void gate_sums_kernel(const QuotArgs a) {
  extern __shared__ gl_t sums_stage[];
  const uint32_t grp = G > 1 ? threadIdx.y : 0;
  const uint32_t n = 1u << a.d;
  const uint32_t k = blockIdx.x * blockDim.x + threadIdx.x;
  const uint32_t m = blockIdx.y, r = 2u * m;
  if (k >= n) return;
  const uint32_t ncs = a.NC + a.R;
  const gl_t *csb = a.cs_lde + (size_t)r * ncs * n;
  const gl_t *wlb = a.wires_lde + (size_t)r * a.W * n;
  Consumer out;
  out.ap0 = a.apow;
  out.ap1 = a.apow + a.nterms;
  const uint32_t kb = k * 8u;
  auto W = [&](uint32_t c) { return *(const gl_t *)((const char *)(wlb + (size_t)c * n) + kb); };
  auto LC = [&](uint32_t i) { return *(const gl_t *)((const char *)(csb + (size_t)(a.num_selectors + i) * n) + kb); };
  for (uint32_t gi = 0; gi < a.num_gates; gi++) {
    const GateDesc g = a.gates[gi];
    const uint32_t slot1 = gate_half_slot(g);
    if (!slot1) continue;
    if (G > 1 && gate_sums_group(g) != grp) continue;
    out.acc0.clear();
    out.acc1.clear();
    out.t = a.K + a.K * a.nchunks;
    eval_gate<BaseOps, false>(g, W, LC, a.pi_hash, c_poseidon_rc, out);
    if constexpr (STAGE) {
      const uint32_t rb = blockDim.x, sk = (slot1 - 1) * a.K;
      sums_stage[sk * rb + threadIdx.x] = out.acc0.value();
      if (a.K > 1) sums_stage[(sk + 1) * rb + threadIdx.x] = out.acc1.value();
    } else {
      gl_t *h = a.hsum + ((size_t)m * a.nsk + (size_t)(slot1 - 1) * a.K) * n + k;
      h[0] = out.acc0.value();
      if (a.K > 1) h[n] = out.acc1.value();
    }
  }
  if constexpr (STAGE) {
    for (uint32_t gi = 0; gi < a.num_gates; gi++) {
      const GateDesc g = a.gates[gi];
      const uint32_t slot1 = gate_half_slot(g);
      if (!slot1 || (G > 1 && gate_sums_group(g) != grp)) continue;
      const uint32_t rb = blockDim.x, sk = (slot1 - 1) * a.K;
      gl_t *h = a.hsum + ((size_t)m * a.nsk + sk) * n + k;
      h[0] = sums_stage[sk * rb + threadIdx.x];
      if (a.K > 1) h[n] = sums_stage[(sk + 1) * rb + threadIdx.x];
    }
  }
}
struct CrossMat {
  gl_t f[4][4];
};
__global__ __launch_bounds__(256) void gate_sums_cross_kernel(const gl_t *__restrict__ in, const gl_t *__restrict__ inv_scale, gl_t *__restrict__ out,
                                                             uint32_t d, uint32_t cols, CrossMat F) {
  const uint32_t n = 1u << d;
  const uint32_t p = blockIdx.x * blockDim.x + threadIdx.x, col = blockIdx.y;
  if (p >= n) return;
  gl_t P[4];
#pragma unroll
  for (uint32_t m = 0; m < 4; m++) P[m] = gl_mul(in[((size_t)m * cols + col) * n + p], inv_scale[(size_t)(2 * m) * n + p]);
#pragma unroll
  for (uint32_t mo = 0; mo < 4; mo++) {
    Acc160 acc;
    acc.clear();
#pragma unroll
    for (uint32_t m = 0; m < 4; m++) acc.mac(F.f[mo][m], P[m]);
    out[((size_t)mo * cols + col) * n + p] = acc.value();
  }
}
void gate_sums_eval(hipStream_t st, const QuotArgs &a, uint32_t groups) {
  const uint32_t n = 1u << a.d;
  const size_t lds = (size_t)a.nsk * (groups == 4 ? 64 : 256) * sizeof(gl_t);
  static const bool stage_ok = env_flag("P2GPU_SUMS_STAGE", true);
  const bool stage = stage_ok && lds <= 24 * 1024;
  const char *name = groups == 4 ? (stage ? "gate_sums_kernel<4, true>" : "gate_sums_kernel<4, false>") : (stage ? "gate_sums_kernel<1, true>" : "gate_sums_kernel<1, false>");
  ProfScope ps(name, 8.0 * (double)n * 4 * (a.W + a.num_selectors + 1.0 * a.nsk));
  if (groups == 4) {
    if (stage) hipLaunchKernelGGL((gate_sums_kernel<4, true>), dim3(n / 64, 4), dim3(64, 4), lds, st, a);
    else hipLaunchKernelGGL((gate_sums_kernel<4, false>), dim3(n / 64, 4), dim3(64, 4), 0, st, a);
  } else {
    if (stage) hipLaunchKernelGGL((gate_sums_kernel<1, true>), dim3((n + 255) / 256, 4), dim3(256), lds, st, a);
    else hipLaunchKernelGGL((gate_sums_kernel<1, false>), dim3((n + 255) / 256, 4), dim3(256), 0, st, a);
  }
}
void gate_sums_cross(hipStream_t st, const gl_t *in, const gl_t *inv_scale, gl_t *out, uint32_t d, uint32_t cols, const gl_t F[16]) {
  const uint32_t n = 1u << d;
  CrossMat M;
  for (int i = 0; i < 16; i++) M.f[i / 4][i % 4] = F[i];
  ProfScope ps("gate_sums_cross_kernel", 8.0 * (double)n * cols * 8);
  hipLaunchKernelGGL(gate_sums_cross_kernel, dim3((n + 255) / 256, cols), dim3(256), 0, st, in, inv_scale, out, d, cols, M);
}

#ifndef P2_PGATE_WAVES
#define P2_PGATE_WAVES 6
#endif
__global__ __launch_bounds__(256, P2_PGATE_WAVES) void poseidon_gate_kernel(const QuotArgs a, uint32_t gi) {
  const uint32_t n = 1u << a.d;
  const uint32_t k = blockIdx.x * blockDim.x + threadIdx.x;
  const uint32_t z = blockIdx.y;
  const uint32_t r = a.coset_first + z * a.coset_stride;
  if (k >= n) return;
  const GateDesc g = a.gates[gi];
  const uint32_t ncs = a.NC + a.R;
  const gl_t *cs = a.cs_lde + (size_t)r * ncs * n + k;
  const gl_t *wl = a.wires_lde + (size_t)z * a.W * n + k;
// ... 89 lines not shown
```

### acvm-backend-plonky2_amd/csrc/prover.hip

```cpp
#include "prover_internal.hpp"
#include <chrono>

using namespace p2;

namespace {

bool hostprof_on() {
  static const bool on = env_flag("P2GPU_HOSTPROF", false);
  return on;
}

struct Proof {
  const gl_t *wires_dev;
  const uint64_t *pis;
  uint32_t n_pi;
  Challenger ch;
  gl_t pih[4];
  gl_t betas[MAX_CHALLENGES] = {0, 0}, gammas[MAX_CHALLENGES] = {0, 0}, alphas[MAX_CHALLENGES] = {0, 0};
  ext_t zeta;
  Batch *oracles[4];
  std::vector<ext_t> op;
  uint32_t vfirst;
  const uint32_t *h_cls = nullptr;
  const gl_t *h_val = nullptr;
  std::vector<ext_t> final_poly;
  uint64_t pow_witness;
  std::vector<size_t> qidx;
  const gl_t *gathered = nullptr;
  p2gpu_timings T;
  double t_lap;
  Proof(p2gpu_circuit *c, const gl_t *wires_dev_, const uint64_t *pis_, uint32_t n_pi_, double h2d_ms)
      : wires_dev(wires_dev_), pis(pis_), n_pi(n_pi_), oracles{&c->cs, &c->wires, &c->zp, &c->quot}, t_lap(now_ms()) {
    memset(&T, 0, sizeof T);
    T.h2d_ms = h2d_ms;
  }
};

double lap(Proof &P) {
  const double t = now_ms(), dt = t - P.t_lap;
  P.t_lap = t;
  return dt;
}

uint32_t committed_cols(const p2gpu_circuit *c) { return c->NC + c->R + c->W + c->K * (1 + c->PP) + c->K * c->QF; }

int check_public_inputs(const p2gpu_circuit *c, const uint64_t *pis, uint32_t n_pi) {
  if (n_pi != c->num_pi || (n_pi && !pis)) {
    set_err("expected %u public inputs, got %u", c->num_pi, n_pi);
    return P2GPU_E_ARG;
  }
  for (uint32_t i = 0; i < n_pi; i++)
    if (pis[i] >= GL_P) {
      set_err("public input %u is not a canonical field element", i);
      return P2GPU_E_ARG;
    }
  return 0;
}

int commit_wires(p2gpu_circuit *c, Proof &P) {
  g_hp.mark("start");
  TRACE(c, "enter");
  if (int rc = batch_commit_from_values(c, c->wires, P.wires_dev)) return rc;
  TRACE(c, "wires commit");
  return 0;
}

int commit_zs(p2gpu_circuit *c, Proof &P) {
  hipStream_t st = c->stream;
  const uint32_t d = c->d, K = c->K;
  ZsArgs a;
  a.wires = P.wires_dev;
  a.sigmas = c->d_sigmas.p;
  a.k_is = c->d_kis.p;
  a.sub_tw = c->tw_fwd.p;
  a.tw_shift = 0;
  a.d = d; a.R = c->R; a.QF = c->QF; a.nchunks = c->nchunks; a.K = K;
  for (uint32_t k = 0; k < 2; k++) { a.betas[k] = P.betas[k]; a.gammas[k] = P.gammas[k]; }
  a.cp = c->cp.p;
  a.zp = c->zp_vals.p;
  a.sb = d;
  a.row0 = 0;
  a.rows = (uint32_t)c->n;
  uint32_t lgG = 0;
  while ((1u << lgG) < (uint32_t)c->shard_world) lgG++;
  if (c->shard_zs && sharded(c) && (1u << lgG) == (uint32_t)c->shard_world && d >= lgG) {
    a.sb = d - lgG;
    a.rows = (uint32_t)(c->n >> lgG);
    a.row0 = a.rows * (uint32_t)c->shard_rank;
    zs_chunks(st, a);
    const size_t blk = (size_t)K * (c->nchunks + 1) * a.rows;
    if (int rc = shard_allgather(c, c->cp.p + blk * (size_t)c->shard_rank, c->cp.p, blk * sizeof(gl_t))) return rc;
    zs_scan_finish(st, a, c->scan_tmp.p);
  } else {
    zs_partial_products(st, a, c->scan_tmp.p);
  }
  TRACE(c, "zs_partial_products");
  return batch_commit_from_values(c, c->zp, c->zp_vals.p);
}

int commit_quotient(p2gpu_circuit *c, Proof &P) {
  hipStream_t st = c->stream;
  const uint32_t d = c->d, K = c->K, nterms = c->nterms;
  const size_t n = c->n;
  gl_t *ap = c->pin.take<gl_t>((size_t)2 * nterms);
  if (!ap) return pin_exhausted();
  memset(ap, 0, 16 * (size_t)nterms);
  for (uint32_t k = 0; k < K; k++) {
    gl_t a = 1;
    for (uint32_t t = 0; t < nterms; t++) {
      ap[(size_t)k * nterms + t] = a;
      a = gl_mul(a, P.alphas[k]);
    }
  }
  HIP_TRY(hipMemcpyAsync(c->apow.p, ap, 16 * (size_t)nterms, hipMemcpyHostToDevice, st));
  QuotArgs q;
  memset(&q, 0, sizeof q);
  q.cs_lde = c->cs.lde.p;
  q.wires_lde = c->wires.lde.p;
  q.zp_lde = c->zp.lde.p;
  q.k_is = c->d_kis.p;
  q.tw = c->tw_fwd.p;
  q.apow = c->apow.p;
  q.gates = c->d_gates.p;
  q.host_gates = c->gates.data();
  q.out = c->qvals.p;
  q.tw_shift = 0; q.d = d; q.rate_bits = c->rate_bits; q.W = c->W; q.R = c->R; q.NC = c->NC;
  q.num_selectors = c->num_selectors; q.K = K; q.QF = c->QF; q.nchunks = c->nchunks; q.PP = c->PP;
  q.num_gates = c->num_gates; q.nterms = nterms;
  q.coset_first = c->wires.cm.first;
  q.coset_stride = c->wires.cm.stride;
  q.ncosets = c->wires.ncl;
  q.gate_groups = c->gate_groups;
  q.has_poseidon = 0;
  for (auto &g : c->gates)
    if (g.kind == G_POSEIDON) q.has_poseidon = 1;
  for (uint32_t k = 0; k < 2; k++) { q.betas[k] = P.betas[k]; q.gammas[k] = P.gammas[k]; }
  for (int i = 0; i < 4; i++) q.pi_hash[i] = P.pih[i];
  q.qconst = c->qconst.p;
  q.n_inv = gl_inv((gl_t)n);
  q.l0 = c->l0_lde.p;
  q.gate_groups_half = c->gate_groups_half;
  q.nsk = c->half_slots * K;
  q.hsum = c->hsum.p;
  q.use_half = (c->half_gates == 2 || (c->half_gates == 1 && c->half_auto)) && c->half_slots && c->wires.ncl == c->C && c->wires.cm.stride == 1 &&
               c->wires.cm.first == 0;
  if (q.use_half) {
    const size_t per = (size_t)4 * q.nsk * n;
    gate_sums_eval(st, q, n >= 64 ? c->sums_groups : 1u);
    ntt_batch(st, c->plan_inv, c->hsum.p, c->htmp_a.p, 4 * q.nsk, 1, nullptr, q.n_inv, false);
    gate_sums_cross(st, c->htmp_a.p, c->inv_scale.p, c->htmp_b.p, d, q.nsk, c->half_cross);
    CosetMap odd;
    odd.first = 1;
    odd.stride = 2;
    ntt_batch(st, c->plan_fwd, c->htmp_b.p, c->hsum.p + per, q.nsk, 4, c->scale.p, 1, true, odd);
    TRACE(c, "gate sums (half domain)");
  }
  quotient_eval(st, q);
  TRACE(c, "quotient_eval");
  ntt_batch(st, c->plan_inv, c->qvals.p, c->qtmp.p, K * c->wires.ncl, 1, nullptr, q.n_inv, false);
  const gl_t *pr = c->qtmp.p;
  if (sharded(c)) {
    if (int rc = shard_allgather(c, c->qtmp.p, c->qvals.p, (size_t)K * c->wires.ncl * n * sizeof(gl_t))) return rc;
    pr = c->qvals.p;
  }
  const gl_t wC = gl_root(c->rate_bits), gn = gl_pow(GL_GEN, n);
  quotient_chunks(st, pr, c->inv_scale.p, c->quot.coeffs.p, d, K, c->rate_bits, gl_inv(wC), gl_inv(gn), gl_inv((gl_t)c->C),
                  (uint32_t)c->shard_world);
  TRACE(c, "quotient_chunks");
  return batch_commit_from_coeffs(c, c->quot);
}

int open_at_zeta(p2gpu_circuit *c, Proof &P) {
  hipStream_t st = c->stream;
  const uint32_t d = c->d, K = c->K, W = c->W, nall = committed_cols(c);
  const size_t n = c->n;
  ext_t zn = P.zeta;
  for (uint32_t i = 0; i < d; i++) zn = ext_mul(zn, zn);
  if (ext_eq(zn, ext_from(1))) {
    set_err("Opening point is in the subgroup.");
    return P2GPU_E_OPENING_IN_SUBGROUP;
  }
  P.op.resize(nall + K);
  uint32_t parts = 1;
  while (parts < 16 && (n / (parts * 2)) >= 1024) parts *= 2;
  ext_powers_bitrev2(st, P.zeta, ext_scale(P.zeta, gl_root(d)), d, c->pw.p, c->pw.p + 2 * n);
  const bool structured = batch_colnz(c, c->wires) != nullptr;
  const ColHints wh = structured ? wire_hints(c, 0, false) : ColHints();
  if (structured) {
    compact_nonzero(st, c->wire_nz.p, c->W, c->wire_nzlist.p);
    if (c->sparse_coeffs.p) eval_columns(st, c->sparse_coeffs.p, 1, d, c->pw.p, parts, c->sparse_partial.p);
  }
  size_t base = 0;
  EvalSegs es;
  for (int o = 0; o < 4; o++) {
    if (structured && P.oracles[o] == &c->wires) {
      es.hinted = es.count;
      es.cls = wh.cls;
      es.val = wh.val;
      es.basis_partial = c->sparse_partial.p;
    }
    es.seg[es.count++] = {P.oracles[o]->coeffs.p, c->pw.p, c->partial.p + base * parts * 2, P.oracles[o]->cols};
    base += P.oracles[o]->cols;
  }
  es.seg[es.count++] = {c->zp.coeffs.p, c->pw.p + 2 * n, c->partial.p + base * parts * 2, K};
  if (sharded(c) && c->shard_world > 1) {
    const uint32_t total = (uint32_t)(nall + K), G = (uint32_t)c->shard_world, cpr = (total + G - 1) / G;
    eval_columns_multi(st, es, d, parts, cpr * (uint32_t)c->shard_rank, cpr);
    const size_t blk = (size_t)cpr * parts * 2;
    if (int rc = shard_allgather(c, c->partial.p + blk * (size_t)c->shard_rank, c->partial.p, blk * 8)) return rc;
  } else {
    eval_columns_multi(st, es, d, parts);
  }
  const size_t npart = (size_t)(nall + K) * parts * 2;
  gl_t *part = c->pin.take<gl_t>(npart);
  if (!part) return pin_exhausted();
  HIP_TRY(hipMemcpyAsync(part, c->partial.p, npart * 8, hipMemcpyDeviceToHost, st));
  uint32_t *dense_count = structured ? c->pin.take<uint32_t>(1) : nullptr;
  if (dense_count) HIP_TRY(hipMemcpyAsync(dense_count, c->wire_nzlist.p, 4, hipMemcpyDeviceToHost, st));
  if (P.vfirst != UINT32_MAX) {
    uint32_t *hc = c->pin.take<uint32_t>(W);
    gl_t *hv = c->pin.take<gl_t>(W);
    if (!hc || !hv) return pin_exhausted();
    HIP_TRY(hipMemcpyAsync(hc, c->wire_nz.p, 4 * (size_t)W, hipMemcpyDeviceToHost, st));
    HIP_TRY(hipMemcpyAsync(hv, c->wire_scalar.p, 8 * (size_t)W, hipMemcpyDeviceToHost, st));
    P.h_cls = hc;
    P.h_val = hv;
  }
  g_hp.mark("enq(openings)");
  if (int rc_ = wait_stream(c)) return rc_;
  g_hp.mark("WAIT(openings)");
  if (dense_count && (uint64_t)(c->W - *dense_count) * 20u < c->W) c->structured_off = true;
  if (dense_count) c->last_dense = *dense_count;
  for (size_t j = 0; j < nall + K; j++) {
    gl_t a0 = 0, a1 = 0;
    for (uint32_t p = 0; p < parts; p++) {
      a0 = gl_add(a0, part[(j * parts + p) * 2]);
      a1 = gl_add(a1, part[(j * parts + p) * 2 + 1]);
    }
    P.op[j] = ext_make(a0, a1);
  }
  TRACE(c, "openings");
  return 0;
}

int fri_reduce(p2gpu_circuit *c, Proof &P, ext_t alpha) {
  hipStream_t st = c->stream;
  const uint32_t d = c->d, K = c->K, nall = committed_cols(c);
  const size_t n = c->n;
  gl_t *apw = c->pin.take<gl_t>((size_t)2 * nall);
  if (!apw) return pin_exhausted();
  ext_t a = ext_from(1);
  ext_t f0z = ext_from(0), f1z = ext_from(0);
  for (uint32_t j = 0; j < nall; j++) {
    apw[2 * j] = a.c0;
    apw[2 * j + 1] = a.c1;
    f0z = ext_add(f0z, ext_mul(a, P.op[j]));
    if (j < K) f1z = ext_add(f1z, ext_mul(a, P.op[nall + j]));
    a = ext_mul(a, alpha);
  }
  HIP_TRY(hipMemcpyAsync(c->ext_apow.p, apw, 16 * (size_t)nall, hipMemcpyHostToDevice, st));
  gl_t *F0 = c->f01.p, *F1 = c->f01.p + 2 * n;
  uint32_t j0 = 0;
  bool reduced = false;
  if (c->shard_reduce && sharded(c)) {
    const uint32_t G = (uint32_t)c->shard_world, cpr = (nall + G - 1) / G;
    const uint32_t c0 = std::min(cpr * (uint32_t)c->shard_rank, nall), c1 = std::min(c0 + cpr, nall);
    bool first = true;
    uint32_t jo = 0;
    for (int o = 0; o < 4; o++) {
      const uint32_t co = P.oracles[o]->cols;
      const uint32_t lo = std::max(c0, jo) - jo, hi = std::min(c1, jo + co) > jo ? std::min(c1, jo + co) - jo : 0;
      if (hi > lo) {
        reduce_columns(st, P.oracles[o]->coeffs.p + (size_t)lo * n, hi - lo, d, c->ext_apow.p, jo + lo, F0, !first);
        first = false;
      }
      jo += co;
    }
    if (first) HIP_TRY(hipMemsetAsync(F0, 0, 16 * n, st));
    if (int rc = shard_allgather(c, F0, c->xchg_recv.p, 16 * n)) return rc;
    sum_parts(st, c->xchg_recv.p, G, 2 * n, F0);
    reduced = true;
  }
  for (int o = reduced ? 4 : 0; o < 4; o++) {
    const bool hw = batch_colnz(c, *P.oracles[o]) != nullptr;
    const bool unit = hw && c->sparse_coeffs.p != nullptr;
    if (unit) class1_fold(st, wire_hints(c, 0, false), c->W, c->ext_apow.p, j0, c->sparse_partial.p + 32);
    reduce_columns(st, P.oracles[o]->coeffs.p, P.oracles[o]->cols, d, c->ext_apow.p, j0, F0, o != 0,
                   hw ? c->wire_nzlist.p : nullptr, unit ? c->sparse_coeffs.p : nullptr, unit ? c->sparse_partial.p + 32 : nullptr);
    j0 += P.oracles[o]->cols;
// ... 509 lines not shown
```

### acvm-backend-plonky2_amd/csrc/selftest.hip

```cpp
#include "internal.hpp"

namespace p2 {

__global__ void field_selftest_kernel(const uint64_t *a, const uint64_t *b, uint32_t n, unsigned long long *bad) {
  const uint32_t i = blockIdx.x * blockDim.x + threadIdx.x;
  if (i >= n) return;
  const uint64_t x = a[i], y = b[i];
  const gl_t xc = gl_canon_c(x), yc = gl_canon_c(y);
  if (gl_canon(x) != xc) atomicAdd(&bad[0], 1ULL);
  if (gl_add(xc, yc) != gl_add_c(xc, yc)) atomicAdd(&bad[1], 1ULL);
  if (gl_sub(xc, yc) != gl_sub_c(xc, yc)) atomicAdd(&bad[2], 1ULL);
  if (gl_reduce128(x, y) != gl_reduce128_c(x, y)) atomicAdd(&bad[3], 1ULL);
  const uint64_t plo = xc * yc, phi = __umul64hi(xc, yc);
  const gl_t prod = gl_reduce128_c(plo, phi);
  if (gl_mul(xc, yc) != prod) atomicAdd(&bad[4], 1ULL);
  {
    uint64_t lo = plo + xc, hi = phi + (lo < xc);
    if (gl_mul_add(xc, yc, xc) != gl_reduce128_c(lo, hi)) atomicAdd(&bad[5], 1ULL);
  }
  gl_t pw = 1;
  bool ok = true;
  static_for<1, 96>([&](auto ec) {
    constexpr int e = decltype(ec)::value;
    pw = gl_add_c(pw, pw);
    const uint64_t l = xc * pw, h = __umul64hi(xc, pw);
    if (mul_pow2<e>(xc) != gl_reduce128_c(l, h)) ok = false;
  });
  if (!ok) atomicAdd(&bad[6], 1ULL);
  {
    Acc160 acc;
    acc.clear();
    acc.mac(xc, yc);
    acc.mac(yc, yc);
    acc.mac(xc, xc);
    const uint64_t l2 = yc * yc, h2 = __umul64hi(yc, yc), l3 = xc * xc, h3 = __umul64hi(xc, xc);
    const gl_t want = gl_add_c(gl_add_c(prod, gl_reduce128_c(l2, h2)), gl_reduce128_c(l3, h3));
    if (acc.value() != want) atomicAdd(&bad[7], 1ULL);
  }
  if (gl_canon(gl_mul_nc(x, y)) != prod) atomicAdd(&bad[8], 1ULL);
  {
    uint64_t lo = plo + xc, hi = phi + (lo < xc);
    if (gl_canon(gl_mul_add_nc(x, yc, xc)) != gl_reduce128_c(lo, hi)) atomicAdd(&bad[9], 1ULL);
  }
  if (gl_canon(gl_reduce128_nc(x, y)) != gl_reduce128_c(x, y)) atomicAdd(&bad[10], 1ULL);
  if (gl_canon(gl_add(x, yc)) != gl_add_c(xc, yc) || gl_add(xc, yc) != gl_add_c(xc, yc)) atomicAdd(&bad[11], 1ULL);
  if (gl_canon(gl_sub(x, yc)) != gl_sub_c(xc, yc) || gl_sub(xc, yc) != gl_sub_c(xc, yc)) atomicAdd(&bad[12], 1ULL);
  {
    const uint64_t u = gl_mul_nc(x, y), v = gl_mul_add_nc(y, xc, yc);
    const uint64_t w = gl_mul_nc(u, v);
    uint64_t l2 = plo + yc, h2 = phi + (l2 < yc);
    const gl_t vv = gl_reduce128_c(l2, h2);
    const uint64_t l3 = prod * vv, h3 = __umul64hi(prod, vv);
    if (gl_canon(w) != gl_reduce128_c(l3, h3)) atomicAdd(&bad[13], 1ULL);
    if (gl_canon(gl_add(w, xc)) != gl_add_c(gl_reduce128_c(l3, h3), xc)) atomicAdd(&bad[13], 1ULL);
    if (gl_canon(gl_sub(w, xc)) != gl_sub_c(gl_reduce128_c(l3, h3), xc)) atomicAdd(&bad[13], 1ULL);
  }
}
void field_selftest(hipStream_t st, const uint64_t *a, const uint64_t *b, uint32_t n, unsigned long long *bad) {
  hipLaunchKernelGGL(field_selftest_kernel, dim3((n + 255) / 256), dim3(256), 0, st, a, b, n, bad);
}

__global__ void bitrev_cols_kernel(const gl_t *in, gl_t *out, uint32_t d, uint32_t cols) {
  uint32_t p = blockIdx.x * blockDim.x + threadIdx.x;
  uint32_t c = blockIdx.y;
  if (p >= (1u << d)) return;
  out[((size_t)c << d) + bitrev32(p, d)] = in[((size_t)c << d) + p];
}
void bitrev_cols(hipStream_t st, const gl_t *in, gl_t *out, uint32_t d, uint32_t cols) {
  uint32_t n = 1u << d;
  hipLaunchKernelGGL(bitrev_cols_kernel, dim3((n + 255) / 256, cols), dim3(256), 0, st, in, out, d, cols);
}

}
```

### acvm-backend-plonky2_amd/prover.py

```python
import ctypes
import os

import numpy as np

_HERE = os.path.dirname(os.path.abspath(__file__))
_LIB = None

UINT64_MAX = (1 << 64) - 1


class P2GpuError(RuntimeError):
    def __init__(self, code, msg):
        super().__init__(f"p2gpu error {code}: {msg}")
        self.code = code


class _Timings(ctypes.Structure):
    _fields_ = [
        ("wires_commit_ms", ctypes.c_double),
        ("zs_commit_ms", ctypes.c_double),
        ("quotient_ms", ctypes.c_double),
        ("openings_ms", ctypes.c_double),
        ("fri_ms", ctypes.c_double),
        ("total_ms", ctypes.c_double),
        ("h2d_ms", ctypes.c_double),
        ("pow_witness", ctypes.c_uint64),
    ]


_ALLGATHER_FN = ctypes.CFUNCTYPE(ctypes.c_int, ctypes.c_void_p, ctypes.c_uint64, ctypes.c_uint64, ctypes.c_uint64)


class _DevBytes:

    def __init__(self, ptr, nbytes):
        self.__cuda_array_interface__ = {"shape": (int(nbytes),), "typestr": "|u1", "data": (int(ptr), False),
                                         "version": 2}


def lib_path():
    return os.environ.get("P2GPU_LIBRARY") or os.path.join(_HERE, "libp2gpu.so")


def load_library():
    global _LIB
    if _LIB is not None:
        return _LIB
    path = lib_path()
    if not os.path.exists(path):
        raise P2GpuError(-8, f"{path} is missing: build it with __graft_entry__.build() (hipcc, gfx950)")
    try:
        import torch
    except Exception:
        pass
    lib = ctypes.CDLL(path)
    vp, sz, u8p = ctypes.c_void_p, ctypes.c_size_t, ctypes.c_void_p
    lib.p2gpu_last_error.restype = ctypes.c_char_p
    lib.p2gpu_init.argtypes = [ctypes.POINTER(ctypes.c_int), ctypes.c_int]
    lib.p2gpu_circuit_create.argtypes = [u8p, sz, ctypes.POINTER(vp)]
    lib.p2gpu_circuit_destroy.argtypes = [vp]
    lib.p2gpu_circuit_destroy.restype = None
    lib.p2gpu_circuit_cap.argtypes = [vp, u8p]
    lib.p2gpu_circuit_digest.argtypes = [vp, u8p]
    lib.p2gpu_proof_size_bound.argtypes = [vp]
    lib.p2gpu_proof_size_bound.restype = sz
    lib.p2gpu_circuit_device.argtypes = [vp]
    lib.p2gpu_circuit_hash_bytes.argtypes = [vp]
    lib.p2gpu_prove.argtypes = [vp, vp, vp, ctypes.c_uint32, u8p, ctypes.POINTER(sz), ctypes.POINTER(_Timings)]
    lib.p2gpu_prove_dev.argtypes = lib.p2gpu_prove.argtypes
    lib.p2gpu_prove_routed.argtypes = lib.p2gpu_prove.argtypes
    a = lib.p2gpu_prove.argtypes
    lib.p2gpu_prove_sparse.argtypes = [a[0], a[1], ctypes.c_uint32, ctypes.c_void_p, ctypes.c_uint32] + list(a[2:])
    lib.p2gpu_fill_witness.argtypes = [vp, vp]
    lib.p2gpu_witness_plan_create.argtypes = [vp, vp, sz, ctypes.POINTER(vp)]
    lib.p2gpu_witness_plan_build.argtypes = [vp, vp, sz, ctypes.POINTER(vp)]
    lib.p2gpu_witness_plan_export.argtypes = [vp, vp, vp, vp, vp]
    lib.p2gpu_witness_plan_create_gen.argtypes = [vp, vp, sz, vp, sz, ctypes.POINTER(vp)]
    lib.p2gpu_witness_plan_build_gen.argtypes = [vp, vp, sz, vp, sz, ctypes.POINTER(vp)]
    lib.p2gpu_witness_plan_export_generators.argtypes = [vp, vp, ctypes.POINTER(sz)]
    lib.p2gpu_witness_plan_destroy.argtypes = [vp]
    lib.p2gpu_witness_plan_destroy.restype = None
    lib.p2gpu_witness_plan_info.argtypes = [vp, vp, vp]
    lib.p2gpu_generate_witness.argtypes = [vp, vp, vp]
    lib.p2gpu_generate_witness_batch.argtypes = [vp, vp, sz, vp, vp, vp]
    lib.p2gpu_prove_seeds.argtypes = [vp, vp, vp, ctypes.c_uint32, u8p, ctypes.POINTER(sz), ctypes.POINTER(_Timings)]
    lib.p2gpu_verify.argtypes = [vp, u8p, sz]
    lib.p2gpu_circuit_export_vk.argtypes = [vp, u8p, ctypes.POINTER(sz)]
    lib.p2gpu_circuit_export_vk_plonky2.argtypes = [vp, u8p, ctypes.POINTER(sz)]
    lib.p2gpu_verifier_create_plonky2.argtypes = [u8p, sz, ctypes.c_int, ctypes.POINTER(vp)]
    lib.p2gpu_verifier_create.argtypes = [u8p, sz, ctypes.POINTER(vp)]
    lib.p2gpu_proof_compress.argtypes = [vp, u8p, sz, u8p, ctypes.POINTER(sz)]
    lib.p2gpu_proof_decompress.argtypes = [vp, u8p, sz, u8p, ctypes.POINTER(sz)]
    lib.p2gpu_verify_compressed.argtypes = [vp, u8p, sz]
    lib.p2gpu_circuit_set.argtypes = [vp, ctypes.c_char_p, ctypes.c_uint64]
    lib.p2gpu_circuit_set_shard.argtypes = [vp, ctypes.c_int, ctypes.c_int, _ALLGATHER_FN, vp]
    lib.p2gpu_shard_unique_id.argtypes = [vp]
    lib.p2gpu_circuit_set_shard_rccl.argtypes = [vp, ctypes.c_int, ctypes.c_int, vp]
    lib.p2gpu_kernel_stats.argtypes = [vp, ctypes.c_char_p, vp, vp, vp, ctypes.c_int]
    lib.p2gpu_ifft_batch.argtypes = [vp, sz, ctypes.c_uint, vp]
    lib.p2gpu_lde_batch.argtypes = [vp, sz, ctypes.c_uint, ctypes.c_uint, vp]
    lib.p2gpu_commit_values.argtypes = [vp, sz, ctypes.c_uint, ctypes.c_uint, ctypes.c_uint, u8p]
    lib.p2gpu_hash_rows.argtypes = [vp, sz, sz, u8p]
    lib.p2gpu_field_selftest.argtypes = [vp, vp, sz, vp]
    lib.p2gpu_field_selftest16.argtypes = [vp, vp, sz, vp]
    lib.p2gpu_device_info.argtypes = [ctypes.c_char_p, sz, ctypes.POINTER(ctypes.c_int), ctypes.POINTER(sz)]
    lib.p2gpu_peer_access.argtypes = [ctypes.POINTER(ctypes.c_int), ctypes.c_int]
    lib.p2gpu_circuit_create_on.argtypes = [u8p, sz, ctypes.c_int, ctypes.POINTER(vp)]
    lib.p2gpu_circuit_build.argtypes = [vp, vp, ctypes.c_uint32, vp, vp, vp, sz, ctypes.c_uint32, ctypes.POINTER(vp)]
    lib.p2gpu_circuit_build_on.argtypes = [vp, vp, ctypes.c_uint32, vp, vp, vp, sz, ctypes.c_uint32, ctypes.c_int, ctypes.POINTER(vp)]
    lib.p2gpu_circuit_export_blob.argtypes = [vp, u8p, ctypes.POINTER(sz)]
    lib.p2gpu_peer_access.restype = ctypes.c_int
    lib.p2gpu_host_alloc.argtypes = [sz]
    lib.p2gpu_host_alloc.restype = vp
    lib.p2gpu_host_free.argtypes = [vp]
    lib.p2gpu_host_free.restype = None
    _LIB = lib
    return lib


def _check(rc):
    if rc != 0:
        raise P2GpuError(rc, load_library().p2gpu_last_error().decode(errors="replace"))


def _u64(a):
    a = np.ascontiguousarray(a, dtype=np.uint64)
    return a


def init(devices=(0,)):
    lib = load_library()
    devs = (ctypes.c_int * len(devices))(*[int(d) for d in devices])
    _check(lib.p2gpu_init(devs, len(devices)))


class _HostBlock:

    def __init__(self, nbytes):
        self._lib = load_library()
        self.ptr = self._lib.p2gpu_host_alloc(nbytes)
        if not self.ptr:
            raise P2GpuError(-3, self._lib.p2gpu_last_error().decode(errors="replace"))
        self.buf = (ctypes.c_uint8 * max(1, nbytes)).from_address(self.ptr)

    def __del__(self):
        if getattr(self, "ptr", None):
            self.buf = None
            self._lib.p2gpu_host_free(self.ptr)
            self.ptr = None


def host_array(shape, dtype=np.uint64):
    shape = (shape,) if isinstance(shape, int) else tuple(shape)
    nbytes = int(np.prod(shape, dtype=np.int64)) * np.dtype(dtype).itemsize
    blk = _HostBlock(nbytes)
    arr = np.frombuffer(blk.buf, dtype=dtype, count=nbytes // np.dtype(dtype).itemsize).reshape(shape)
    _HOST_BLOCKS[id(blk)] = blk
    arr.flags.writeable = True
    return arr


_HOST_BLOCKS = {}


def host_free(arr):
    addr = arr.ctypes.data
    for k, blk in list(_HOST_BLOCKS.items()):
        if blk.ptr == addr:
            del _HOST_BLOCKS[k]
            blk.__del__()
            return
    raise P2GpuError(-1, "host_free: not an array from host_array")


def device_info():
    lib = load_library()
    name = ctypes.create_string_buffer(256)
    cu = ctypes.c_int()
    mem = ctypes.c_size_t()
    _check(lib.p2gpu_device_info(name, 256, ctypes.byref(cu), ctypes.byref(mem)))
    return {"name": name.value.decode(), "cu_count": cu.value, "hbm_bytes": mem.value}


def peer_access():
    lib = load_library()
    n = lib.p2gpu_peer_access(None, 0)
    if n < 0:
        _check(n)
    m = (ctypes.c_int * (n * n))()
    _check(min(0, lib.p2gpu_peer_access(m, n * n)))
    return [[int(m[a * n + b]) for b in range(n)] for a in range(n)]


class ProofWithPublicInputs:

    def __init__(self, data, timings=None):
        self._data = bytes(data)
        self.timings = timings or {}

    def to_bytes(self):
        return self._data

    def __len__(self):
        return len(self._data)

    def __eq__(self, other):
        return isinstance(other, ProofWithPublicInputs) and self._data == other._data


class CircuitData:

    def __init__(self, blob, device=None):
        lib = load_library()
        self._lib = lib
        self._blob = np.ascontiguousarray(np.frombuffer(blob, dtype=np.uint8) if not isinstance(blob, np.ndarray) else blob)
        hdr = self._blob[:256].view(np.uint32)
        self.degree_bits = int(hdr[2])
        self.num_wires = int(hdr[3])
        self.num_routed_wires = int(hdr[4])
        self.rate_bits = int(hdr[9])
        self.cap_height = int(hdr[10])
        self.num_public_inputs = int(hdr[24])
        self._h = ctypes.c_void_p()
        if device is None:
            _check(lib.p2gpu_circuit_create(self._blob.ctypes.data, self._blob.nbytes, ctypes.byref(self._h)))
        else:
            _check(lib.p2gpu_circuit_create_on(self._blob.ctypes.data, self._blob.nbytes, int(device), ctypes.byref(self._h)))
        self._bound = lib.p2gpu_proof_size_bound(self._h)

    @classmethod
    def from_blob(cls, blob):
        return cls(blob)

    @classmethod
    def build(cls, degree_bits, gates, row_gate, row_constants, copies, num_public_inputs=0, num_wires=234, num_routed_wires=80,
              num_challenges=2, quotient_degree_factor=8, rate_bits=3, cap_height=4, proof_of_work_bits=16, num_query_rounds=28,
              hasher=0, device=None):
        lib = load_library()
        bp, gd, rg, rc, cp = _build_args(degree_bits, gates, row_gate, row_constants, copies, num_public_inputs, num_wires, num_routed_wires,
                                         num_challenges, quotient_degree_factor, rate_bits, cap_height, proof_of_work_bits, num_query_rounds)
        self = cls.__new__(cls)
        self._lib = lib
        self._blob = None
        self.degree_bits, self.num_wires, self.num_routed_wires = int(degree_bits), int(num_wires), int(num_routed_wires)
        self.rate_bits, self.cap_height, self.num_public_inputs = int(rate_bits), int(cap_height), int(num_public_inputs)
        self._h = ctypes.c_void_p()
        args = [ctypes.byref(bp), gd, len(gates), rg.ctypes.data, rc.ctypes.data if rc.size else None, cp.ctypes.data if cp.size else None,
                len(cp), int(hasher)]
        if device is None:
            _check(lib.p2gpu_circuit_build(*args, ctypes.byref(self._h)))
        else:
            _check(lib.p2gpu_circuit_build_on(*args, int(device), ctypes.byref(self._h)))
        self._bound = lib.p2gpu_proof_size_bound(self._h)
        return self

    def to_blob(self):
        ln = ctypes.c_size_t(0)
# ... 337 lines not shown
        _check(self._lib.p2gpu_circuit_export_vk_plonky2(self._h, out.ctypes.data, ctypes.byref(n)))
        return out[:n.value].tobytes()


CircuitData.compress = _ProofFormats.compress
CircuitData.decompress = _ProofFormats.decompress
CircuitData.verify_compressed = _ProofFormats.verify_compressed
CircuitData.to_plonky2_vk_bytes = _ProofFormats.to_plonky2_bytes


class VerifierCircuitData(_ProofFormats):

    def __init__(self, blob):
        lib = load_library()
        self._lib = lib
        self._blob = np.ascontiguousarray(np.frombuffer(blob, dtype=np.uint8))
        self._h = ctypes.c_void_p()
        _check(lib.p2gpu_verifier_create(self._blob.ctypes.data, self._blob.nbytes, ctypes.byref(self._h)))
        self._read_header()

    @classmethod
    def from_plonky2_bytes(cls, vk, hasher=0):
        self = cls.__new__(cls)
        lib = load_library()
        self._lib = lib
        buf = np.ascontiguousarray(np.frombuffer(bytes(vk), dtype=np.uint8))
        self._h = ctypes.c_void_p()
        _check(lib.p2gpu_verifier_create_plonky2(buf.ctypes.data if buf.size else None, buf.size, int(hasher), ctypes.byref(self._h)))
        n = ctypes.c_size_t(0)
        _check(lib.p2gpu_circuit_export_vk(self._h, None, ctypes.byref(n)))
        self._blob = np.zeros(n.value, dtype=np.uint8)
        _check(lib.p2gpu_circuit_export_vk(self._h, self._blob.ctypes.data, ctypes.byref(n)))
        self._read_header()
        return self

    def _read_header(self):
        hdr = self._blob[:256].view(np.uint32)
        self.degree_bits = int(hdr[2])
        self.cap_height = int(hdr[10])
        self.num_public_inputs = int(hdr[24])

    def to_bytes(self):
        return self._blob.tobytes()

    def hash_bytes(self):
        return int(self._lib.p2gpu_circuit_hash_bytes(self._h))

    def circuit_digest(self):
        out = np.zeros(self.hash_bytes(), dtype=np.uint8)
        _check(self._lib.p2gpu_circuit_digest(self._h, out.ctypes.data))
        return out.tobytes()

    def constants_sigmas_cap(self):
        out = np.zeros(self.hash_bytes() << self.cap_height, dtype=np.uint8)
        _check(self._lib.p2gpu_circuit_cap(self._h, out.ctypes.data))
        return out.tobytes()

    def verify(self, proof):
        _verify(self._lib, self._h, proof)

    def close(self):
        if getattr(self, "_h", None) and self._h.value:
            self._lib.p2gpu_circuit_destroy(self._h)
            self._h = ctypes.c_void_p()

    def __del__(self):
        try:
            self.close()
        except Exception:
            pass


class _BuildParams(ctypes.Structure):
    _fields_ = [(k, ctypes.c_uint32) for k in ("degree_bits", "num_wires", "num_routed_wires", "num_challenges", "quotient_degree_factor",
                                                "rate_bits", "cap_height", "proof_of_work_bits", "num_query_rounds", "num_public_inputs")]


class _GateDecl(ctypes.Structure):
    _fields_ = [("kind", ctypes.c_uint32), ("p", ctypes.c_uint32 * 4), ("degree", ctypes.c_uint32), ("num_constants", ctypes.c_uint32)]


def _build_args(degree_bits, gates, row_gate, row_constants, copies, num_public_inputs, num_wires, num_routed_wires, num_challenges,
                quotient_degree_factor, rate_bits, cap_height, proof_of_work_bits, num_query_rounds):
    bp = _BuildParams(degree_bits, num_wires, num_routed_wires, num_challenges, quotient_degree_factor, rate_bits, cap_height,
                      proof_of_work_bits, num_query_rounds, num_public_inputs)
    gd = (_GateDecl * len(gates))()
    for i, (kind, ps, deg, nk) in enumerate(gates):
        gd[i].kind, gd[i].degree, gd[i].num_constants = kind, deg, nk
        for j, v in enumerate(tuple(ps) + (0,) * (4 - len(ps))):
            gd[i].p[j] = v
    rg = np.ascontiguousarray(row_gate, dtype=np.uint32)
    rc = np.ascontiguousarray(row_constants, dtype=np.uint64)
    cp = np.ascontiguousarray(copies, dtype=np.uint32).reshape(-1, 4)
    if rg.size != 1 << degree_bits:
        raise P2GpuError(-7, "row_gate must have 2^degree_bits entries")
    return bp, gd, rg, rc, cp


def build_blob(degree_bits, gates, row_gate, row_constants, copies, num_public_inputs=0, num_wires=234, num_routed_wires=80,
               num_challenges=2, quotient_degree_factor=8, rate_bits=3, cap_height=4, proof_of_work_bits=16, num_query_rounds=28):
    lib = load_library()
    lib.p2gpu_build_blob.argtypes = [ctypes.c_void_p, ctypes.c_void_p, ctypes.c_uint32, ctypes.c_void_p, ctypes.c_void_p, ctypes.c_void_p,
                                     ctypes.c_size_t, ctypes.c_void_p, ctypes.POINTER(ctypes.c_size_t)]
    bp, gd, rg, rc, cp = _build_args(degree_bits, gates, row_gate, row_constants, copies, num_public_inputs, num_wires, num_routed_wires,
                                     num_challenges, quotient_degree_factor, rate_bits, cap_height, proof_of_work_bits, num_query_rounds)
    ln = ctypes.c_size_t(0)
    args = [ctypes.byref(bp), gd, len(gates), rg.ctypes.data, rc.ctypes.data if rc.size else None, cp.ctypes.data if cp.size else None, len(cp)]
    _check(lib.p2gpu_build_blob(*args, None, ctypes.byref(ln)))
    out = np.zeros(ln.value, dtype=np.uint8)
    _check(lib.p2gpu_build_blob(*args, out.ctypes.data, ctypes.byref(ln)))
    return out[:ln.value]


def ifft_batch(vals):
    lib = load_library()
    v = _u64(vals)
    ncols, n = v.shape
    d = n.bit_length() - 1
    out = np.zeros_like(v)
    _check(lib.p2gpu_ifft_batch(v.ctypes.data, ncols, d, out.ctypes.data))
    return out


def lde_batch(coeffs, rate_bits=3):
    lib = load_library()
    c = _u64(coeffs)
    ncols, n = c.shape
    d = n.bit_length() - 1
    out = np.zeros((ncols, n << rate_bits), dtype=np.uint64)
    _check(lib.p2gpu_lde_batch(c.ctypes.data, ncols, d, rate_bits, out.ctypes.data))
    return out


def commit_values(vals, rate_bits=3, cap_height=4):
    lib = load_library()
    v = _u64(vals)
    ncols, n = v.shape
    d = n.bit_length() - 1
    out = np.zeros(25 << cap_height, dtype=np.uint8)
    _check(lib.p2gpu_commit_values(v.ctypes.data, ncols, d, rate_bits, cap_height, out.ctypes.data))
    return out.tobytes()


def field_selftest(a, b):
    lib = load_library()
    x = np.ascontiguousarray(a, dtype=np.uint64)
    y = np.ascontiguousarray(b, dtype=np.uint64)
    assert x.shape == y.shape and x.ndim == 1
    bad = np.zeros(16, dtype=np.uint64)
    _check(lib.p2gpu_field_selftest16(x.ctypes.data, y.ctypes.data, x.size, bad.ctypes.data))
    return bad


def hash_rows(rows):
    lib = load_library()
    r = _u64(rows)
    n_rows, row_len = r.shape
    out = np.zeros(25 * n_rows, dtype=np.uint8)
    _check(lib.p2gpu_hash_rows(r.ctypes.data, n_rows, row_len, out.ctypes.data))
    return out.reshape(n_rows, 25)
```

### include/p2gpu.h

```cpp
#ifndef P2GPU_H
#define P2GPU_H
#include <stddef.h>
#include <stdint.h>

#ifdef __cplusplus
extern "C" {
#endif

#define P2GPU_OK 0
#define P2GPU_E_BLOB -1
#define P2GPU_E_BUFFER -2
#define P2GPU_E_DEVICE -3
#define P2GPU_E_OPENING_IN_SUBGROUP -4
#define P2GPU_E_UNSATISFIED -5
#define P2GPU_E_CAP_MISMATCH -6
#define P2GPU_E_ARG -7
#define P2GPU_E_NOT_INIT -8
#define P2GPU_E_VERIFY -9

typedef struct p2gpu_circuit p2gpu_circuit;

typedef struct {
  double wires_commit_ms;
  double zs_commit_ms;
  double quotient_ms;
  double openings_ms;
  double fri_ms;
  double total_ms;
  double h2d_ms;
  uint64_t pow_witness;
} p2gpu_timings;

int p2gpu_init(const int *device_ids, int n_devices);
void *p2gpu_host_alloc(size_t bytes);
void p2gpu_host_free(void *p);

int p2gpu_circuit_create(const uint8_t *blob, size_t len, p2gpu_circuit **out);
int p2gpu_circuit_create_on(const uint8_t *blob, size_t len, int device_id, p2gpu_circuit **out);
void p2gpu_circuit_destroy(p2gpu_circuit *c);
int p2gpu_circuit_hash_bytes(const p2gpu_circuit *c);
int p2gpu_circuit_cap(const p2gpu_circuit *c, uint8_t *out);
int p2gpu_circuit_digest(const p2gpu_circuit *c, uint8_t *out);
int p2gpu_circuit_device(const p2gpu_circuit *c);
size_t p2gpu_proof_size_bound(const p2gpu_circuit *c);

int p2gpu_prove(p2gpu_circuit *c, const uint64_t *wires, const uint64_t *public_inputs, uint32_t n_pi,
                uint8_t *proof_out, size_t *proof_len, p2gpu_timings *opt_timings);
int p2gpu_prove_dev(p2gpu_circuit *c, const uint64_t *wires_dev, const uint64_t *public_inputs, uint32_t n_pi,
                    uint8_t *proof_out, size_t *proof_len, p2gpu_timings *opt_timings);
int p2gpu_fill_witness(p2gpu_circuit *c, uint64_t *wires_dev);
int p2gpu_prove_routed(p2gpu_circuit *c, const uint64_t *routed, const uint64_t *public_inputs, uint32_t n_pi,
                       uint8_t *proof_out, size_t *proof_len, p2gpu_timings *opt_timings);
int p2gpu_prove_sparse(p2gpu_circuit *c, const uint64_t *wires, uint32_t ncols, const uint64_t *tail, uint32_t row,
                       const uint64_t *public_inputs, uint32_t n_pi, uint8_t *proof_out, size_t *proof_len,
                       p2gpu_timings *opt_timings);

typedef struct p2gpu_witness_plan p2gpu_witness_plan;
int p2gpu_witness_plan_create(p2gpu_circuit *c, const uint32_t *seed_cells , size_t n_seeds,
                              p2gpu_witness_plan **out);
int p2gpu_witness_plan_build(p2gpu_circuit *c, const uint32_t *seed_cells , size_t n_seeds,
                             p2gpu_witness_plan **out);
#define P2GPU_GEN_EQUALITY 0
typedef struct { uint32_t kind; uint32_t cells[4][2];  } p2gpu_generator;
int p2gpu_witness_plan_create_gen(p2gpu_circuit *c, const uint32_t *seed_cells, size_t n_seeds,
                                  const p2gpu_generator *generators, size_t n_generators, p2gpu_witness_plan **out);
int p2gpu_witness_plan_build_gen(p2gpu_circuit *c, const uint32_t *seed_cells, size_t n_seeds,
                                 const p2gpu_generator *generators, size_t n_generators, p2gpu_witness_plan **out);
int p2gpu_witness_plan_export_generators(const p2gpu_witness_plan *p, uint32_t *table, size_t *n_generators);
int p2gpu_witness_plan_export(const p2gpu_witness_plan *p, uint32_t *cell_slot, uint64_t *ops, uint32_t *level_off, size_t sizes[3]);
void p2gpu_witness_plan_destroy(p2gpu_witness_plan *p);
int p2gpu_witness_plan_info(const p2gpu_witness_plan *p, uint64_t counts[5], double ms[2]);
int p2gpu_generate_witness(p2gpu_witness_plan *p, const uint64_t *seed_values, uint64_t *wires_dev_out);
int p2gpu_generate_witness_batch(p2gpu_witness_plan *p, const uint64_t *seed_values , size_t batch,
                                 uint64_t *wires_dev_out ,
                                 int *status ,
                                 uint32_t *bad_cells );
int p2gpu_prove_seeds(p2gpu_witness_plan *p, const uint64_t *seed_values, const uint64_t *public_inputs, uint32_t n_pi,
                      uint8_t *proof_out, size_t *proof_len, p2gpu_timings *opt_timings);

typedef struct {
  uint32_t degree_bits, num_wires, num_routed_wires, num_challenges, quotient_degree_factor, rate_bits, cap_height,
      proof_of_work_bits, num_query_rounds, num_public_inputs;
} p2gpu_build_params;
typedef struct {
  uint32_t kind, p[4], degree, num_constants;
} p2gpu_gate_decl;
int p2gpu_build_blob(const p2gpu_build_params *params, const p2gpu_gate_decl *gates, uint32_t num_gates, const uint32_t *row_gate,
                     const uint64_t *row_constants, const uint32_t *copies, size_t num_copies, uint8_t *blob_out,
                     size_t *blob_len);

int p2gpu_circuit_build(const p2gpu_build_params *params, const p2gpu_gate_decl *gates, uint32_t num_gates, const uint32_t *row_gate,
                        const uint64_t *row_constants, const uint32_t *copies, size_t num_copies, uint32_t hasher, p2gpu_circuit **out);
int p2gpu_circuit_build_on(const p2gpu_build_params *params, const p2gpu_gate_decl *gates, uint32_t num_gates, const uint32_t *row_gate,
                           const uint64_t *row_constants, const uint32_t *copies, size_t num_copies, uint32_t hasher, int device_id,
                           p2gpu_circuit **out);
int p2gpu_circuit_export_blob(const p2gpu_circuit *c, uint8_t *out, size_t *len);

int p2gpu_verify(const p2gpu_circuit *c, const uint8_t *proof, size_t len);
int p2gpu_circuit_export_vk(const p2gpu_circuit *c, uint8_t *out, size_t *len);
int p2gpu_verifier_create(const uint8_t *blob, size_t len, p2gpu_circuit **out);
int p2gpu_circuit_export_vk_plonky2(const p2gpu_circuit *c, uint8_t *out, size_t *len);
int p2gpu_verifier_create_plonky2(const uint8_t *vk, size_t len, int hasher, p2gpu_circuit **out);

int p2gpu_proof_compress(const p2gpu_circuit *c, const uint8_t *proof, size_t len, uint8_t *out, size_t *out_len);
int p2gpu_proof_decompress(const p2gpu_circuit *c, const uint8_t *cproof, size_t len, uint8_t *out, size_t *out_len);
int p2gpu_verify_compressed(const p2gpu_circuit *c, const uint8_t *cproof, size_t len);

int p2gpu_circuit_set(p2gpu_circuit *c, const char *key, uint64_t value);
int p2gpu_kernel_stats(p2gpu_circuit *c, char *names, double *ms, double *bytes, uint64_t *launches, int cap);

typedef int (*p2gpu_allgather_fn)(void *ctx, uint64_t send_dev, uint64_t recv_dev, uint64_t bytes_per_rank);
int p2gpu_circuit_set_shard(p2gpu_circuit *c, int rank, int world, p2gpu_allgather_fn fn, void *ctx);
int p2gpu_shard_unique_id(uint8_t id_out[128]);
int p2gpu_shard_assemble_cap(int world, unsigned rate_bits, unsigned cap_h, const uint8_t *gathered, uint8_t *cap_out);
int p2gpu_circuit_set_shard_rccl(p2gpu_circuit *c, int rank, int world, const uint8_t id[128]);

int p2gpu_ifft_batch(const uint64_t *vals, size_t ncols, unsigned d, uint64_t *coeffs_out);
int p2gpu_lde_batch(const uint64_t *coeffs, size_t ncols, unsigned d, unsigned rate_bits, uint64_t *lde_out);
int p2gpu_commit_values(const uint64_t *vals, size_t ncols, unsigned d, unsigned rate_bits, unsigned cap_h,
                        uint8_t *cap_out);
int p2gpu_hash_rows(const uint64_t *rows, size_t n_rows, size_t row_len, uint8_t *digests_out);
int p2gpu_field_selftest(const uint64_t *a, const uint64_t *b, size_t n, uint64_t bad_out[8]);
int p2gpu_field_selftest16(const uint64_t *a, const uint64_t *b, size_t n, uint64_t bad_out[16]);

const char *p2gpu_last_error(void);
int p2gpu_device_info(char *name_out, size_t name_cap, int *cu_count, size_t *hbm_bytes);
int p2gpu_peer_access(int *matrix_out, int cap);

#ifdef __cplusplus
}
#endif
#endif
```

Baseline: 235.5 proofs/sec.

## Rescale permutation argument terms by inverse beta and use powers-of-7 coset shifts

In the quotient evaluation, each permutation factor (w + beta*k*x + gamma) is divided by beta, giving w*b' + g' + k*x with b' = 1/beta and g' = gamma/beta. The numerator and denominator then share one multiply-add and each need only an addition. The dropped beta^chunk factors are folded into the host-side alpha power weights. When the k_is form a powers-of-7 chain, k_j*x is stepped with a cheap multiply-by-7 shift-subtract instead of a full field multiply. The aim is fewer 64-bit modular multiplies per routed wire in the hot quotient kernel, at the cost of extra host pow/inv work and non-canonical intermediate values that need care.

Result: no change. 235.6 proofs/sec (median of 3 runs) (+0.0%).

```diff
diff --git a/acvm-backend-plonky2_amd/__init__.py b/acvm-backend-plonky2_amd/__init__.py
--- a/acvm-backend-plonky2_amd/__init__.py
+++ b/acvm-backend-plonky2_amd/__init__.py
@@ -15,6 +15,8 @@
     commit_values,
     hash_rows,
     field_selftest,
+    perm_prims_selftest,
+    perm_selftest,
     lib_path,
     load_library,
 )
diff --git a/acvm-backend-plonky2_amd/csrc/circuit.hpp b/acvm-backend-plonky2_amd/csrc/circuit.hpp
--- a/acvm-backend-plonky2_amd/csrc/circuit.hpp
+++ b/acvm-backend-plonky2_amd/csrc/circuit.hpp
@@ -192,6 +192,8 @@
   uint32_t gate_groups_half = 1;
   uint32_t sums_groups = 1;
   int half_gates = 1;
+  int perm_form = 1;
+  bool kis_pow7 = false;
   bool half_auto = false;
   gl_t half_cross[16];
   DBuf<gl_t> hsum, htmp_a, htmp_b;
diff --git a/acvm-backend-plonky2_amd/csrc/gl.hpp b/acvm-backend-plonky2_amd/csrc/gl.hpp
--- a/acvm-backend-plonky2_amd/csrc/gl.hpp
+++ b/acvm-backend-plonky2_amd/csrc/gl.hpp
@@ -131,7 +131,7 @@
 P2_HD gl_t gl_reduce128(uint64_t lo, uint64_t hi) {
   return gl_reduce_words((uint32_t)lo, (uint32_t)(lo >> 32), (uint32_t)hi, (uint32_t)(hi >> 32));
 }
-P2_HD gl_t gl_reduce_add_eps(uint32_t w0, uint32_t w1, uint32_t w2) {
+P2_HD uint64_t gl_reduce_add_eps_nc(uint32_t w0, uint32_t w1, uint32_t w2) {
   uint32_t r0, r1, t0, t1;
   uint64_t k;
   asm("v_sub_co_u32 %2, vcc, 0, %7\n\t"
@@ -144,7 +144,21 @@
       : "=&v"(r0), "=&v"(r1), "=&v"(t0), "=&v"(t1), "=&s"(k)
       : "v"(w0), "v"(w1), "v"(w2)
       : "vcc", "scc");
-  return gl_canon(gl_join(r0, r1));
+  return gl_join(r0, r1);
+}
+P2_HD gl_t gl_reduce_add_eps(uint32_t w0, uint32_t w1, uint32_t w2) { return gl_canon(gl_reduce_add_eps_nc(w0, w1, w2)); }
+P2_HD uint64_t gl_add_nc(uint64_t a, gl_t b) {
+  uint32_t s0, s1;
+  uint64_t k;
+  asm("v_add_co_u32 %0, vcc, %3, %5\n\t"
+      "v_addc_co_u32 %1, vcc, %4, %6, vcc\n\t"
+      "v_subb_co_u32 %0, %2, %0, 0, vcc\n\t"
+      P2_HZ_A "s_andn2_b64 vcc, vcc, %2\n\t" P2_HZ_B
+      "v_addc_co_u32 %1, vcc, %1, 0, vcc"
+      : "=&v"(s0), "=&v"(s1), "=&s"(k)
+      : "v"((uint32_t)a), "v"((uint32_t)(a >> 32)), "v"((uint32_t)b), "v"((uint32_t)(b >> 32))
+      : "vcc", "scc");
+  return gl_join(s0, s1);
 }
 P2_HD gl_t gl_reduce_eps_sub(uint32_t z, uint32_t h0, uint32_t h1) {
   uint32_t r0, r1, t0, t1;
@@ -166,7 +180,23 @@
 P2_HD gl_t gl_add(gl_t a, gl_t b) { return gl_add_c(a, b); }
 P2_HD gl_t gl_sub(gl_t a, gl_t b) { return gl_sub_c(a, b); }
 P2_HD gl_t gl_reduce128(uint64_t lo, uint64_t hi) { return gl_reduce128_c(lo, hi); }
-#endif
+P2_HD uint64_t gl_add_nc(uint64_t a, gl_t b) {
+  uint64_t s = a + b;
+  if (s < a) s += GL_EPS;
+  return s;
+}
+P2_HD uint64_t gl_reduce_add_eps_nc(uint32_t w0, uint32_t w1, uint32_t w2) {
+  const uint64_t e = ((uint64_t)w2 << 32) - w2;
+  uint64_t s = (((uint64_t)w1 << 32) | w0) + e;
+  if (s < e) s += GL_EPS;
+  return s;
+}
+#endif
+P2_HD uint64_t gl_mul7_nc(uint64_t t) {
+  const uint64_t lo = t << 3, r = lo - t;
+  const uint32_t H = (uint32_t)(t >> 61) - (uint32_t)(lo < t);
+  return gl_reduce_add_eps_nc((uint32_t)r, (uint32_t)(r >> 32), H);
+}
 #if defined(__HIPCC__)
 template <class T>
 __device__ __forceinline__ T ld_uniform(const T *p) {
diff --git a/acvm-backend-plonky2_amd/csrc/handle.hip b/acvm-backend-plonky2_amd/csrc/handle.hip
--- a/acvm-backend-plonky2_amd/csrc/handle.hip
+++ b/acvm-backend-plonky2_amd/csrc/handle.hip
@@ -118,6 +118,8 @@
 
 void schedule_gates(p2gpu_circuit *c) {
   c->nterms = c->K + c->K * c->nchunks + c->max_gate_constraints;
+  c->perm_form = env_flag("P2GPU_PERM_FORM", true) ? 1 : 0;
+  c->kis_pow7 = kis_are_pow7(c->k_is.data(), c->R);
   auto cost = [](const GateDesc &g) { return g.kind == G_POSEIDON ? 0u : 4u * g.num_constraints + 8u; };
   const uint32_t perm_cost = (uint32_t)env_uint("P2GPU_PERM_COST", 8u * c->R + 100u);
   uint32_t total = 0;
@@ -691,6 +693,7 @@
   else if (k == "shard_reduce") c->shard_reduce = (int)value;
   else if (k == "shard_zs") c->shard_zs = (int)value;
   else if (k == "half_gates") c->half_gates = (int)value;
+  else if (k == "perm_form") c->perm_form = (int)value;
   else if (k == "blocking_sync") c->blocking_sync = (int)value;
   else if (k == "virtual_columns") {
     c->virtual_columns = (int)value;
@@ -877,6 +880,69 @@
   field_selftest(S.st, da, db, (uint32_t)n, bad);
   HIP_TRY(hipMemcpyAsync(bad_out, bad, 8 * words, hipMemcpyDeviceToHost, S.st));
   HIP_TRY(hipStreamSynchronize(S.st));
+  return P2GPU_OK;
+} P2GPU_CATCH
+
+int p2gpu_perm_prims_selftest(const uint64_t *a, const uint64_t *b, size_t n, uint64_t bad_out[4]) try {
+  if (int rc = ensure_device()) return rc;
+  if (!a || !b || !bad_out || n == 0 || n > ((size_t)1 << 28)) return P2GPU_E_ARG;
+  Scratch S;
+  HIP_TRY(hipStreamCreate(&S.st));
+  uint64_t *da = S.alloc<uint64_t>(n), *db = S.alloc<uint64_t>(n);
+  unsigned long long *bad = S.alloc<unsigned long long>(4);
+  if (!da || !db || !bad) { set_err("hipMalloc failed"); return P2GPU_E_DEVICE; }
+  HIP_TRY(hipMemcpyAsync(da, a, 8 * n, hipMemcpyHostToDevice, S.st));
+  HIP_TRY(hipMemcpyAsync(db, b, 8 * n, hipMemcpyHostToDevice, S.st));
+  HIP_TRY(hipMemsetAsync(bad, 0, 32, S.st));
+  perm_prims_selftest(S.st, da, db, (uint32_t)n, bad);
+  HIP_TRY(hipMemcpyAsync(bad_out, bad, 32, hipMemcpyDeviceToHost, S.st));
+  HIP_TRY(hipStreamSynchronize(S.st));
+  return P2GPU_OK;
+} P2GPU_CATCH
+
+int p2gpu_perm_selftest(const uint64_t *w, const uint64_t *sigma, const uint64_t *x, const uint64_t *prev, const uint64_t *next,
+                        const uint64_t *k, size_t cnt, size_t rows, size_t K, const uint64_t *betas, const uint64_t *gammas,
+                        int perm_form, uint64_t *out, uint64_t info_out[2]) try {
+  if (int rc = ensure_device()) return rc;
+  if (!w || !sigma || !x || !prev || !next || !k || !betas || !gammas || !out || !info_out || cnt == 0 || cnt > MAX_ROUTED || rows == 0 ||
+      rows > ((size_t)1 << 20) || K == 0 || K > MAX_CHALLENGES)
+    return P2GPU_E_ARG;
+  auto canonical = [](const uint64_t *v, size_t m) {
+    for (size_t i = 0; i < m; i++)
+      if (v[i] >= GL_P) return false;
+    return true;
+  };
+  if (!canonical(w, cnt * rows) || !canonical(sigma, cnt * rows) || !canonical(x, rows) || !canonical(prev, K * rows) || !canonical(next, K * rows) ||
+      !canonical(k, cnt) || !canonical(betas, K) || !canonical(gammas, K)) {
+    set_err("p2gpu_perm_selftest: every input is a canonical field element");
+    return P2GPU_E_ARG;
+  }
+  Scratch S;
+  HIP_TRY(hipStreamCreate(&S.st));
+  PermSelftestArgs a;
+  memset(&a, 0, sizeof a);
+  auto up = [&](const uint64_t *h, size_t m) -> gl_t * {
+    gl_t *dv = S.alloc<gl_t>(m);
+    if (dv && hipMemcpyAsync(dv, h, 8 * m, hipMemcpyHostToDevice, S.st) != hipSuccess) return nullptr;
+    return dv;
+  };
+  a.w = up(w, cnt * rows);
+  a.sigma = up(sigma, cnt * rows);
+  a.x = up(x, rows);
+  a.prev = up(prev, K * rows);
+  a.next = up(next, K * rows);
+  a.k = up(k, cnt);
+  a.out = S.alloc<gl_t>(4 * K * rows);
+  if (!a.w || !a.sigma || !a.x || !a.prev || !a.next || !a.k || !a.out) { set_err("hipMalloc / copy failed"); return P2GPU_E_DEVICE; }
+  a.cnt = (uint32_t)cnt; a.rows = (uint32_t)rows; a.K = (uint32_t)K;
+  for (size_t c = 0; c < K; c++) { a.betas[c] = betas[c]; a.gammas[c] = gammas[c]; }
+  a.pc = perm_consts(a.betas, a.gammas, a.K, perm_form != 0, kis_are_pow7(k, a.cnt));
+  for (size_t c = 0; c < K; c++) a.weight[c] = a.pc.form ? gl_pow(a.betas[c], cnt) : 1;
+  perm_chunk_selftest(S.st, a);
+  HIP_TRY(hipMemcpyAsync(out, a.out, 8 * 4 * K * rows, hipMemcpyDeviceToHost, S.st));
+  HIP_TRY(hipStreamSynchronize(S.st));
+  info_out[0] = a.pc.form;
+  info_out[1] = a.pc.pow7;
   return P2GPU_OK;
 } P2GPU_CATCH
 
diff --git a/acvm-backend-plonky2_amd/csrc/internal.hpp b/acvm-backend-plonky2_amd/csrc/internal.hpp
--- a/acvm-backend-plonky2_amd/csrc/internal.hpp
+++ b/acvm-backend-plonky2_amd/csrc/internal.hpp
@@ -103,6 +103,26 @@
 bool tree_levels(hipStream_t st, dig_t *lvl, uint32_t cosets, uint32_t m, uint32_t cap_per, const gl_t *prc = nullptr,
                  dig_t *host_mirror = nullptr);
 
+struct PermConsts {
+  gl_t b[MAX_CHALLENGES], g[MAX_CHALLENGES];
+  uint32_t form;
+  uint32_t pow7;
+};
+inline bool kis_are_pow7(const gl_t *k_is, uint32_t R) {
+  for (uint32_t j = 0; j + 1 < R; j++)
+    if (k_is[j + 1] != gl_mul(k_is[j], 7)) return false;
+  return true;
+}
+inline PermConsts perm_consts(const gl_t *betas, const gl_t *gammas, uint32_t K, bool on, bool pow7) {
+  PermConsts pc = {{0, 0}, {0, 0}, on ? 1u : 0u, pow7 ? 1u : 0u};
+  for (uint32_t c = 0; c < K; c++)
+    if (betas[c] == 0) pc.form = 0;
+  for (uint32_t c = 0; c < K && pc.form; c++) {
+    pc.b[c] = gl_inv(betas[c]);
+    pc.g[c] = gl_mul(gammas[c], pc.b[c]);
+  }
+  return pc;
+}
 struct ZsArgs {
   const gl_t *wires;
   const gl_t *sigmas;
@@ -138,12 +158,26 @@
   gl_t *hsum;
   uint32_t coset_first, coset_stride, ncosets;
   gl_t betas[MAX_CHALLENGES], gammas[MAX_CHALLENGES];
+  PermConsts pc;
   gl_t pi_hash[4];
   const gl_t *qconst;
   gl_t n_inv;
   const gl_t *l0;
 };
 void quotient_eval(hipStream_t st, const QuotArgs &a);
+void perm_prims_selftest(hipStream_t st, const uint64_t *a, const uint64_t *b, uint32_t n, unsigned long long *bad);
+struct PermSelftestArgs {
+  const gl_t *w, *sigma;
+  const gl_t *x;
+  const gl_t *prev, *next;
+  const gl_t *k;
+  uint32_t cnt, rows, K;
+  gl_t betas[MAX_CHALLENGES], gammas[MAX_CHALLENGES];
+  PermConsts pc;
+  gl_t weight[MAX_CHALLENGES];
+  gl_t *out;
+};
+void perm_chunk_selftest(hipStream_t st, const PermSelftestArgs &a);
 void gate_sums_eval(hipStream_t st, const QuotArgs &a, uint32_t groups);
 void gate_sums_cross(hipStream_t st, const gl_t *in, const gl_t *inv_scale, gl_t *out, uint32_t d, uint32_t cols, const gl_t F[16]);
 void fill_l0_table(hipStream_t st, const gl_t *qconst, const gl_t *tw, uint32_t tw_shift, uint32_t d, uint32_t cosets, gl_t n_inv, gl_t *out);
diff --git a/acvm-backend-plonky2_amd/csrc/permarg.hpp b/acvm-backend-plonky2_amd/csrc/permarg.hpp
--- /dev/null
+++ b/acvm-backend-plonky2_amd/csrc/permarg.hpp
@@ -0,0 +1,84 @@
+#pragma once
+#include "internal.hpp"
+
+namespace p2 {
+
+struct PermProd {
+  uint64_t n0, d0, n1, d1;
+};
+
+template <class LW, class LS>
+__device__ __forceinline__ PermProd perm_chunk8(uint32_t j0, uint32_t j1, uint32_t K, const gl_t *k_is, const gl_t *betas, const gl_t *gammas,
+                                                gl_t bx0, gl_t bx1, LW w, LS s) {
+  PermProd p;
+  p.n1 = 1;
+  p.d1 = 1;
+  {
+    const gl_t wv = w(j0);
+    const gl_t sg = s(j0);
+    const gl_t kj = k_is[j0];
+    const gl_t wg0 = gl_add(wv, gammas[0]);
+    p.n0 = gl_mul_add_nc(bx0, kj, wg0);
+    p.d0 = gl_mul_add_nc(betas[0], sg, wg0);
+    if (K > 1) {
+      const gl_t wg1 = gl_add(wv, gammas[1]);
+      p.n1 = gl_mul_add_nc(bx1, kj, wg1);
+      p.d1 = gl_mul_add_nc(betas[1], sg, wg1);
+    }
+  }
+#pragma unroll 7
+  for (uint32_t j = j0 + 1; j < j1; j++) {
+    const gl_t wv = w(j);
+    const gl_t sg = s(j);
+    const gl_t kj = k_is[j];
+    const gl_t wg0 = gl_add(wv, gammas[0]);
+    p.n0 = gl_mul_nc(p.n0, gl_mul_add_nc(bx0, kj, wg0));
+    p.d0 = gl_mul_nc(p.d0, gl_mul_add_nc(betas[0], sg, wg0));
+    if (K > 1) {
+      const gl_t wg1 = gl_add(wv, gammas[1]);
+      p.n1 = gl_mul_nc(p.n1, gl_mul_add_nc(bx1, kj, wg1));
+      p.d1 = gl_mul_nc(p.d1, gl_mul_add_nc(betas[1], sg, wg1));
+    }
+  }
+  return p;
+}
+
+template <bool POW7, class LW, class LS>
+__device__ __forceinline__ PermProd perm_chunk6(uint32_t j0, uint32_t j1, uint32_t K, const gl_t *k_is, const PermConsts &pc, gl_t x, gl_t &t,
+                                                LW w, LS s) {
+  PermProd p;
+  p.n1 = 1;
+  p.d1 = 1;
+  {
+    const gl_t wv = w(j0);
+    const gl_t sg = s(j0);
+    const gl_t tj = POW7 ? t : gl_mul(k_is[j0], x);
+    const uint64_t u0 = gl_mul_add_nc(wv, pc.b[0], pc.g[0]);
+    p.n0 = gl_add_nc(u0, tj);
+    p.d0 = gl_add_nc(u0, sg);
+    if (K > 1) {
+      const uint64_t u1 = gl_mul_add_nc(wv, pc.b[1], pc.g[1]);
+      p.n1 = gl_add_nc(u1, tj);
+      p.d1 = gl_add_nc(u1, sg);
+    }
+    if (POW7) t = gl_canon(gl_mul7_nc(tj));
+  }
+#pragma unroll 7
+  for (uint32_t j = j0 + 1; j < j1; j++) {
+    const gl_t wv = w(j);
+    const gl_t sg = s(j);
+    const gl_t tj = POW7 ? t : gl_mul(k_is[j], x);
+    const uint64_t u0 = gl_mul_add_nc(wv, pc.b[0], pc.g[0]);
+    p.n0 = gl_mul_nc(p.n0, gl_add_nc(u0, tj));
+    p.d0 = gl_mul_nc(p.d0, gl_add_nc(u0, sg));
+    if (K > 1) {
+      const uint64_t u1 = gl_mul_add_nc(wv, pc.b[1], pc.g[1]);
+      p.n1 = gl_mul_nc(p.n1, gl_add_nc(u1, tj));
+      p.d1 = gl_mul_nc(p.d1, gl_add_nc(u1, sg));
+    }
+    if (POW7) t = gl_canon(gl_mul7_nc(tj));
+  }
+  return p;
+}
+
+}
diff --git a/acvm-backend-plonky2_amd/csrc/plonk.hip b/acvm-backend-plonky2_amd/csrc/plonk.hip
--- a/acvm-backend-plonky2_amd/csrc/plonk.hip
+++ b/acvm-backend-plonky2_amd/csrc/plonk.hip
@@ -1,5 +1,6 @@
 #include "internal.hpp"
 #include "gates.hpp"
+#include "permarg.hpp"
 
 namespace p2 {
 
@@ -22,28 +23,7 @@
   const uint32_t cols = a.K * (a.nchunks + 1);
   return ((((size_t)(i >> a.sb) * cols + col) << a.sb) | (i & ((1u << a.sb) - 1u)));
 }
-__global__ __launch_bounds__(256) void zs_chunk_kernel(ZsArgs a) {
-  const uint32_t n = 1u << a.d;
-  const uint32_t i = a.row0 + blockIdx.x * blockDim.x + threadIdx.x;
-  const uint32_t c = blockIdx.y;
-  if (i >= a.row0 + a.rows) return;
-  const gl_t x = root_pow(a.sub_tw, a.tw_shift, a.d, i);
-  const gl_t beta = a.betas[c], gamma = a.gammas[c];
-  const gl_t bx = gl_mul(beta, x);
-  gl_t np[16], dp[16];
-  for (uint32_t m = 0; m < a.nchunks; m++) {
-    uint64_t pn = 1, pd = 1;
-    for (uint32_t j = m * a.QF; j < (m + 1) * a.QF && j < a.R; j++) {
-      gl_t wv = a.wires[(size_t)j * n + i];
-      const gl_t wg = gl_add(wv, gamma);
-      const uint64_t num = gl_mul_add_nc(bx, a.k_is[j], wg);
-      const uint64_t den = gl_mul_add_nc(beta, a.sigmas[(size_t)j * n + i], wg);
-      pn = gl_mul_nc(pn, num);
-      pd = gl_mul_nc(pd, den);
-    }
-    np[m] = gl_canon(pn);
-    dp[m] = gl_canon(pd);
-  }
+__device__ __forceinline__ void zs_row_finish(const ZsArgs &a, uint32_t c, uint32_t i, const gl_t *np, const gl_t *dp) {
   gl_t pre[16];
   gl_t acc = 1;
   for (uint32_t m = 0; m < a.nchunks; m++) {
@@ -60,6 +40,25 @@
     rowp = gl_mul(rowp, q);
   }
   a.cp[zs_idx(a, a.K * a.nchunks + c, i)] = rowp;
+}
+__global__ __launch_bounds__(256) void zs_chunk_kernel(ZsArgs a) {
+  const uint32_t n = 1u << a.d;
+  const uint32_t i = a.row0 + blockIdx.x * blockDim.x + threadIdx.x;
+  const uint32_t c = blockIdx.y;
+  if (i >= a.row0 + a.rows) return;
+  const gl_t x = root_pow(a.sub_tw, a.tw_shift, a.d, i);
+  auto LW = [&](uint32_t j) { return a.wires[(size_t)j * n + i]; };
+  auto LS = [&](uint32_t j) { return a.sigmas[(size_t)j * n + i]; };
+  const gl_t bc[2] = {a.betas[c], 0}, gc[2] = {a.gammas[c], 0};
+  const gl_t bx = gl_mul(bc[0], x);
+  gl_t np[16], dp[16];
+  for (uint32_t m = 0; m < a.nchunks; m++) {
+    const uint32_t j0 = m * a.QF, j1 = min(j0 + a.QF, a.R);
+    const PermProd p = perm_chunk8(j0, j1, 1, a.k_is, bc, gc, bx, 0, LW, LS);
+    np[m] = gl_canon(p.n0);
+    dp[m] = gl_canon(p.d0);
+  }
+  zs_row_finish(a, c, i, np, dp);
 }
 
 __device__ __forceinline__ gl_t block_scan_mul(gl_t v, gl_t *lds, gl_t *total) {
@@ -183,42 +182,26 @@
   const gl_t l0 = a.l0[(size_t)r * n + k];
   for (uint32_t c = 0; c < a.K; c++) out.emit(gl_mul(l0, gl_sub(zl[(size_t)c * n + k], 1)));
   {
-    const gl_t bx0 = gl_mul(a.betas[0], x), bx1 = gl_mul(a.betas[1], x);
+    auto LW = [&](uint32_t j) { return wl[(size_t)j * n]; };
+    auto LS = [&](uint32_t j) { return cs[(size_t)(a.NC + j) * n]; };
+    gl_t bx0 = 0, bx1 = 0, t = 0;
+    if (!a.pc.form) {
+      bx0 = gl_mul(a.betas[0], x);
+      bx1 = gl_mul(a.betas[1], x);
+    } else if (a.pc.pow7) {
+      t = gl_mul(a.k_is[0], x);
+    }
     const uint32_t t_base = out.t;
     for (uint32_t m = 0; m < a.nchunks; m++) {
-      uint64_t n0, d0, n1 = 1, d1 = 1;
-      {
-        const uint32_t j = m * a.QF;
-        const gl_t wv = wl[(size_t)j * n];
-        const gl_t sg = cs[(size_t)(a.NC + j) * n];
-        const gl_t kj = a.k_is[j];
-        const gl_t wg0 = gl_add(wv, a.gammas[0]);
-        n0 = gl_mul_add_nc(bx0, kj, wg0);
-        d0 = gl_mul_add_nc(a.betas[0], sg, wg0);
-        if (a.K > 1) {
-          const gl_t wg1 = gl_add(wv, a.gammas[1]);
-          n1 = gl_mul_add_nc(bx1, kj, wg1);
-          d1 = gl_mul_add_nc(a.betas[1], sg, wg1);
-        }
-      }
-#pragma unroll 7
-      for (uint32_t j = m * a.QF + 1; j < (m + 1) * a.QF && j < a.R; j++) {
-        const gl_t wv = wl[(size_t)j * n];
-        const gl_t sg = cs[(size_t)(a.NC + j) * n];
-        const gl_t kj = a.k_is[j];
-        const gl_t wg0 = gl_add(wv, a.gammas[0]);
-        n0 = gl_mul_nc(n0, gl_mul_add_nc(bx0, kj, wg0));
-        d0 = gl_mul_nc(d0, gl_mul_add_nc(a.betas[0], sg, wg0));
-        if (a.K > 1) {
-          const gl_t wg1 = gl_add(wv, a.gammas[1]);
-          n1 = gl_mul_nc(n1, gl_mul_add_nc(bx1, kj, wg1));
-          d1 = gl_mul_nc(d1, gl_mul_add_nc(a.betas[1], sg, wg1));
-        }
-      }
+      const uint32_t j0 = m * a.QF, j1 = min(j0 + a.QF, a.R);
+      PermProd p;
+      if (!a.pc.form) p = perm_chunk8(j0, j1, a.K, a.k_is, a.betas, a.gammas, bx0, bx1, LW, LS);
+      else if (a.pc.pow7) p = perm_chunk6<true>(j0, j1, a.K, a.k_is, a.pc, x, t, LW, LS);
+      else p = perm_chunk6<false>(j0, j1, a.K, a.k_is, a.pc, x, t, LW, LS);
       for (uint32_t c = 0; c < a.K; c++) {
         const gl_t prev = m == 0 ? zl[(size_t)c * n + k] : zl[((size_t)a.K + c * a.PP + m - 1) * n + k];
         const gl_t next = m == a.nchunks - 1 ? zl[(size_t)c * n + kn] : zl[((size_t)a.K + c * a.PP + m) * n + k];
-        const gl_t term = c == 0 ? gl_sub(gl_mul(prev, n0), gl_mul(next, d0)) : gl_sub(gl_mul(prev, n1), gl_mul(next, d1));
+        const gl_t term = c == 0 ? gl_sub(gl_mul(prev, p.n0), gl_mul(next, p.d0)) : gl_sub(gl_mul(prev, p.n1), gl_mul(next, p.d1));
         out.t = t_base + c * a.nchunks + m;
         out.emit(term);
       }
diff --git a/acvm-backend-plonky2_amd/csrc/prover.hip b/acvm-backend-plonky2_amd/csrc/prover.hip
--- a/acvm-backend-plonky2_amd/csrc/prover.hip
+++ b/acvm-backend-plonky2_amd/csrc/prover.hip
@@ -112,6 +112,16 @@
       a = gl_mul(a, P.alphas[k]);
     }
   }
+  const PermConsts pc = perm_consts(P.betas, P.gammas, K, c->perm_form != 0, c->kis_pow7);
+  if (pc.form)
+    for (uint32_t cc = 0; cc < K; cc++)
+      for (uint32_t m = 0; m < c->nchunks; m++) {
+        const gl_t f = gl_pow(P.betas[cc], std::min(c->QF, c->R - m * c->QF));
+        for (uint32_t k = 0; k < K; k++) {
+          gl_t &w = ap[(size_t)k * nterms + K + cc * c->nchunks + m];
+          w = gl_mul(w, f);
+        }
+      }
   HIP_TRY(hipMemcpyAsync(c->apow.p, ap, 16 * (size_t)nterms, hipMemcpyHostToDevice, st));
   QuotArgs q;
   memset(&q, 0, sizeof q);
@@ -135,6 +145,7 @@
   for (auto &g : c->gates)
     if (g.kind == G_POSEIDON) q.has_poseidon = 1;
   for (uint32_t k = 0; k < 2; k++) { q.betas[k] = P.betas[k]; q.gammas[k] = P.gammas[k]; }
+  q.pc = pc;
   for (int i = 0; i < 4; i++) q.pi_hash[i] = P.pih[i];
   q.qconst = c->qconst.p;
   q.n_inv = gl_inv((gl_t)n);
diff --git a/acvm-backend-plonky2_amd/csrc/selftest.hip b/acvm-backend-plonky2_amd/csrc/selftest.hip
--- a/acvm-backend-plonky2_amd/csrc/selftest.hip
+++ b/acvm-backend-plonky2_amd/csrc/selftest.hip
@@ -1,4 +1,5 @@
 #include "internal.hpp"
+#include "permarg.hpp"
 
 namespace p2 {
 
@@ -60,6 +61,54 @@
   hipLaunchKernelGGL(field_selftest_kernel, dim3((n + 255) / 256), dim3(256), 0, st, a, b, n, bad);
 }
 
+__global__ void perm_prims_selftest_kernel(const uint64_t *a, const uint64_t *b, uint32_t n, unsigned long long *bad) {
+  const uint32_t i = blockIdx.x * blockDim.x + threadIdx.x;
+  if (i >= n) return;
+  const uint64_t x = a[i];
+  const gl_t xc = gl_canon_c(x), yc = gl_canon_c(b[i]);
+  if (gl_canon(gl_add_nc(x, yc)) != gl_add_c(xc, yc)) atomicAdd(&bad[0], 1ULL);
+  gl_t x7 = 0;
+  for (int q = 0; q < 7; q++) x7 = gl_add_c(x7, xc);
+  if (gl_canon(gl_mul7_nc(x)) != x7) atomicAdd(&bad[1], 1ULL);
+  {
+    const uint64_t t1 = gl_mul7_nc(x), t2 = gl_mul7_nc(t1);
+    gl_t x49 = 0;
+    for (int q = 0; q < 7; q++) x49 = gl_add_c(x49, x7);
+    if (gl_canon(t2) != x49) atomicAdd(&bad[2], 1ULL);
+    if (gl_canon(gl_add_nc(t2, yc)) != gl_add_c(x49, yc)) atomicAdd(&bad[2], 1ULL);
+    if (gl_canon(gl_add_nc(gl_add_nc(t1, yc), xc)) != gl_add_c(gl_add_c(x7, yc), xc)) atomicAdd(&bad[2], 1ULL);
+  }
+}
+void perm_prims_selftest(hipStream_t st, const uint64_t *a, const uint64_t *b, uint32_t n, unsigned long long *bad) {
+  hipLaunchKernelGGL(perm_prims_selftest_kernel, dim3((n + 255) / 256), dim3(256), 0, st, a, b, n, bad);
+}
+__global__ void perm_chunk_selftest_kernel(const PermSelftestArgs a) {
+  const uint32_t i = blockIdx.x * blockDim.x + threadIdx.x;
+  if (i >= a.rows) return;
+  const gl_t x = a.x[i];
+  auto LW = [&](uint32_t j) { return a.w[(size_t)j * a.rows + i]; };
+  auto LS = [&](uint32_t j) { return a.sigma[(size_t)j * a.rows + i]; };
+  const gl_t bx0 = gl_mul(a.betas[0], x), bx1 = gl_mul(a.betas[1], x);
+  for (uint32_t f = 0; f < 2; f++) {
+    PermProd p;
+    gl_t t = gl_mul(a.k[0], x);
+    const bool six = f == 1 && a.pc.form;
+    if (!six) p = perm_chunk8(0, a.cnt, a.K, a.k, a.betas, a.gammas, bx0, bx1, LW, LS);
+    else if (a.pc.pow7) p = perm_chunk6<true>(0, a.cnt, a.K, a.k, a.pc, x, t, LW, LS);
+    else p = perm_chunk6<false>(0, a.cnt, a.K, a.k, a.pc, x, t, LW, LS);
+    for (uint32_t c = 0; c < a.K; c++) {
+      const uint64_t N = c ? p.n1 : p.n0, D = c ? p.d1 : p.d0;
+      const gl_t term = gl_sub(gl_mul(a.prev[(size_t)c * a.rows + i], N), gl_mul(a.next[(size_t)c * a.rows + i], D));
+      gl_t *o = a.out + ((size_t)(f * a.K + c) * 2) * a.rows + i;
+      o[0] = six ? gl_mul(term, a.weight[c]) : term;
+      o[a.rows] = gl_mul(gl_canon(N), gl_inv(gl_canon(D)));
+    }
+  }
+}
+void perm_chunk_selftest(hipStream_t st, const PermSelftestArgs &a) {
+  hipLaunchKernelGGL(perm_chunk_selftest_kernel, dim3((a.rows + 63) / 64), dim3(64), 0, st, a);
+}
+
 __global__ void bitrev_cols_kernel(const gl_t *in, gl_t *out, uint32_t d, uint32_t cols) {
   uint32_t p = blockIdx.x * blockDim.x + threadIdx.x;
   uint32_t c = blockIdx.y;
diff --git a/acvm-backend-plonky2_amd/prover.py b/acvm-backend-plonky2_amd/prover.py
--- a/acvm-backend-plonky2_amd/prover.py
+++ b/acvm-backend-plonky2_amd/prover.py
@@ -103,6 +103,8 @@
     lib.p2gpu_hash_rows.argtypes = [vp, sz, sz, u8p]
     lib.p2gpu_field_selftest.argtypes = [vp, vp, sz, vp]
     lib.p2gpu_field_selftest16.argtypes = [vp, vp, sz, vp]
+    lib.p2gpu_perm_prims_selftest.argtypes = [vp, vp, sz, vp]
+    lib.p2gpu_perm_selftest.argtypes = [vp, vp, vp, vp, vp, vp, sz, sz, sz, vp, vp, ctypes.c_int, vp, vp]
     lib.p2gpu_device_info.argtypes = [ctypes.c_char_p, sz, ctypes.POINTER(ctypes.c_int), ctypes.POINTER(sz)]
     lib.p2gpu_peer_access.argtypes = [ctypes.POINTER(ctypes.c_int), ctypes.c_int]
     lib.p2gpu_circuit_create_on.argtypes = [u8p, sz, ctypes.c_int, ctypes.POINTER(vp)]
@@ -746,6 +748,31 @@
     return bad
 
 
+def perm_prims_selftest(a, b):
+    lib = load_library()
+    x = np.ascontiguousarray(a, dtype=np.uint64)
+    y = np.ascontiguousarray(b, dtype=np.uint64)
+    assert x.shape == y.shape and x.ndim == 1
+    bad = np.zeros(4, dtype=np.uint64)
+    _check(lib.p2gpu_perm_prims_selftest(x.ctypes.data, y.ctypes.data, x.size, bad.ctypes.data))
+    return bad
+
+
+def perm_selftest(w, sigma, x, prev, nxt, k, betas, gammas, perm_form=1):
+    lib = load_library()
+    w, sigma, prev, nxt = _u64(w), _u64(sigma), _u64(prev), _u64(nxt)
+    x, k, betas, gammas = (np.ascontiguousarray(v, dtype=np.uint64) for v in (x, k, betas, gammas))
+    cnt, rows = w.shape
+    K = betas.size
+    assert sigma.shape == (cnt, rows) and x.shape == (rows,) and prev.shape == (K, rows) and nxt.shape == (K, rows)
+    assert k.shape == (cnt,) and gammas.shape == (K,)
+    out = np.zeros((2, K, 2, rows), dtype=np.uint64)
+    info = np.zeros(2, dtype=np.uint64)
+    _check(lib.p2gpu_perm_selftest(w.ctypes.data, sigma.ctypes.data, x.ctypes.data, prev.ctypes.data, nxt.ctypes.data, k.ctypes.data,
+                                   cnt, rows, K, betas.ctypes.data, gammas.ctypes.data, int(perm_form), out.ctypes.data, info.ctypes.data))
+    return out, bool(info[0]), bool(info[1])
+
+
 def hash_rows(rows):
     lib = load_library()
     r = _u64(rows)
diff --git a/include/p2gpu.h b/include/p2gpu.h
--- a/include/p2gpu.h
+++ b/include/p2gpu.h
@@ -122,6 +122,10 @@
 int p2gpu_hash_rows(const uint64_t *rows, size_t n_rows, size_t row_len, uint8_t *digests_out);
 int p2gpu_field_selftest(const uint64_t *a, const uint64_t *b, size_t n, uint64_t bad_out[8]);
 int p2gpu_field_selftest16(const uint64_t *a, const uint64_t *b, size_t n, uint64_t bad_out[16]);
+int p2gpu_perm_prims_selftest(const uint64_t *a, const uint64_t *b, size_t n, uint64_t bad_out[4]);
+int p2gpu_perm_selftest(const uint64_t *w, const uint64_t *sigma, const uint64_t *x, const uint64_t *prev, const uint64_t *next,
+                        const uint64_t *k, size_t cnt, size_t rows, size_t K, const uint64_t *betas, const uint64_t *gammas,
+                        int perm_form, uint64_t *out, uint64_t info_out[2]);
 
 const char *p2gpu_last_error(void);
 int p2gpu_device_info(char *name_out, size_t name_cap, int *cu_count, size_t *hbm_bytes);
```
